# sdat2/mSWE-GNN

Measured on AMD Instinct MI355X. Metric: mesh-nodes x rollout-steps / sec (fine-scale nodes); fp32 max-abs err vs CPU ref, higher is better.
Workload: dtype f32

## Files before the change

### mswe-gnn_amd/build_engine.py

```python
import hashlib
import os
import subprocess
import sys
from concurrent.futures import ThreadPoolExecutor

HERE = os.path.dirname(os.path.abspath(__file__))
ROOT = os.path.dirname(HERE)
SRC = ["csrc/kernels_nt1.hip", "csrc/kernels_nt2.hip", "csrc/kernels_nt4.hip",
       "csrc/kernels_common.hip", "csrc/plan.hip", "csrc/metrics.hip", "csrc/floodmaps.hip", "csrc/series.hip",
       "csrc/train.hip"]
HDR = ["csrc/engine.h", "csrc/kernels_impl.h", "csrc/tiling.h", "csrc/graph_build.h", os.path.join(ROOT, "include", "mswegnn.h")]
HDR += sorted(os.path.join("csrc", "kernels", f) for f in os.listdir(os.path.join(HERE, "csrc", "kernels")) if f.endswith(".h"))
ARCH = os.environ.get("MSW_OFFLOAD_ARCH", "gfx950")
FLAGS = ["-O3", "-std=c++17", "-fPIC", f"--offload-arch={ARCH}", "-Wall", "-Wno-unused-result",
         "-I", os.path.join(ROOT, "include")]


def source_hash(variant=""):
    h = hashlib.sha256()
    for f in SRC + HDR:
        path = f if os.path.isabs(f) else os.path.join(HERE, f)
        h.update(os.path.basename(path).encode())
        with open(path, "rb") as fh:
            h.update(fh.read())
    h.update(" ".join(FLAGS + [variant]).replace(ROOT, "<root>").encode())
    return h.hexdigest()


def lib_path(variant=""):
    return os.path.join(HERE, "lib", f"libmswegnn_{variant}.so" if variant else "libmswegnn.so")


def library_matches_sources(variant=""):
    try:
        with open(lib_path(variant) + ".srchash") as f:
            return f.read().strip() == source_hash(variant)
    except OSError:
        return False


def _newer(a, b):
    return not os.path.exists(b) or os.path.getmtime(a) > os.path.getmtime(b)


def build(force=False, verbose=True, variant=""):
    odir = os.path.join(HERE, "_obj" + (f"_{variant}" if variant else ""))
    extra = {"trace": ["-DMSW_TRACE"],
             "valubase": ["-DMSW_PRELU_MAX=0", "-DMSW_EDGE_FULL=0"],
             "nostream": ["-DMSW_STREAM_ST=0"]}.get(variant, [])
    os.makedirs(odir, exist_ok=True)
    os.makedirs(os.path.join(HERE, "lib"), exist_ok=True)
    out = lib_path(variant)
    if os.path.exists(out) and not library_matches_sources(variant):
        force = True
    objs, cmds = [], []
    hdr_t = max(os.path.getmtime(h if os.path.isabs(h) else os.path.join(HERE, h)) for h in HDR)
    for s in SRC:
        src = os.path.join(HERE, s)
        obj = os.path.join(odir, os.path.basename(s) + ".o")
        objs.append(obj)
        stale = force or _newer(src, obj) or (os.path.exists(obj) and hdr_t > os.path.getmtime(obj))
        if stale:
            cmds.append(["hipcc", *FLAGS, *extra, "-c", src, "-o", obj])
    jobs = max(1, min(len(cmds), int(os.environ.get("MAX_JOBS", os.cpu_count() or 1)), 8))
    with ThreadPoolExecutor(jobs) as ex:
        for cmd in cmds:
            if verbose:
                print(" ".join(cmd), flush=True)
        for r in list(ex.map(lambda c: subprocess.run(c, check=False), cmds)):
            if r.returncode != 0:
                raise subprocess.CalledProcessError(r.returncode, r.args)
    if force or any(_newer(o, out) for o in objs):
        cmd = ["hipcc", f"--offload-arch={ARCH}", "-shared", "-fPIC", "-o", out, *objs]
        if verbose:
            print(" ".join(cmd), flush=True)
        subprocess.run(cmd, check=True)
    with open(out + ".srchash", "w") as f:
        f.write(source_hash(variant) + "\n")
    return out


if __name__ == "__main__":
    var = [a[len("--variant="):] for a in sys.argv if a.startswith("--variant=")]
    build(force="--force" in sys.argv, variant="trace" if "--trace" in sys.argv else (var[0] if var else ""))
```

### mswe-gnn_amd/csrc/kernels/k_base.h

```cpp
#pragma once

__device__ __forceinline__ f32x4 ld4(const float* p) { return *reinterpret_cast<const f32x4*>(p); }
__device__ __forceinline__ void st4(float* p, f32x4 v) { *reinterpret_cast<f32x4*>(p) = v; }
#ifndef MSW_STREAM_ST
#define MSW_STREAM_ST 1
#endif
__device__ __forceinline__ void st4_stream(float* p, f32x4 v) {
  if constexpr (MSW_STREAM_ST)
    __builtin_nontemporal_store(v, reinterpret_cast<f32x4*>(p));
  else
    st4(p, v);
}
__device__ __forceinline__ float hsum(f32x4 v) { return (v.x + v.y) + (v.z + v.w); }
__device__ __forceinline__ f32x4 zero4() { return f32x4{0.f, 0.f, 0.f, 0.f}; }

__device__ __forceinline__ float row_sum(float v) {
  const unsigned u = __float_as_uint(v);
  const auto a = __builtin_amdgcn_permlane16_swap(u, u, false, false);
  const float s = __uint_as_float(a[0]) + __uint_as_float(a[1]);
  const unsigned us = __float_as_uint(s);
  const auto b = __builtin_amdgcn_permlane32_swap(us, us, false, false);
  return __uint_as_float(b[0]) + __uint_as_float(b[1]);
}

template <int NT>
__device__ __forceinline__ void normalize_s(f32x4 (&sv)[NT]) {
#pragma clang fp contract(off)
  float ss = 0.f;
#pragma unroll
  for (int t = 0; t < NT; ++t) ss += hsum(sv[t] * sv[t]);
  const float nrm = sqrtf(row_sum(ss));
#pragma unroll
  for (int t = 0; t < NT; ++t) {
    f32x4 q = sv[t] / nrm;
    q.x = (q.x == q.x) ? q.x : 0.f;
    q.y = (q.y == q.y) ? q.y : 0.f;
    q.z = (q.z == q.z) ? q.z : 0.f;
    q.w = (q.w == q.w) ? q.w : 0.f;
    sv[t] = q;
  }
}

__device__ __forceinline__ int wave_id() { return threadIdx.x >> 6; }
__device__ __forceinline__ int logical_block(const Common& c) {
  const int b = blockIdx.x;
  if (c.xcd <= 0) return b;
  const int x = b % kXcds;
  return x < c.xcd ? (b / kXcds) * c.xcd + x : -1;
}
__device__ __forceinline__ int wave_row0() { return (blockIdx.x * kWaves + wave_id()) * kRowsPerWave; }

#ifndef MSW_PRELU_MAX
#define MSW_PRELU_MAX 1
#endif
template <int ACT>
__device__ __forceinline__ float act_static(float x, float slope) {
  if constexpr (ACT == 1) return MSW_PRELU_MAX ? fmaxf(x, slope * x) : (x > 0.f ? x : slope * x);
  else if constexpr (ACT == 8) return x > 0.f ? x : slope * x;
  else if constexpr (ACT == 2) return x > 0.f ? x : 0.f;
  else if constexpr (ACT == 3) return x > 0.f ? x : 0.1f * x;
  else if constexpr (ACT == 4) return x > 0.f ? x : expm1f(x);
  else if constexpr (ACT == 5) return x / (1.f + expf(-x));
  else if constexpr (ACT == 6) return 1.f / (1.f + expf(-x));
  else if constexpr (ACT == 7) return tanhf(x);
  else return x;
}
template <int ACT, int N>
__device__ __forceinline__ void act_tiles_static(f32x4 (&v)[N], float slope) {
  if constexpr (ACT == 1 && MSW_PRELU_MAX) {
#pragma unroll
    for (int t = 0; t < N; ++t) {
      const f32x4 m = v[t] * slope;
#pragma unroll
      for (int r = 0; r < 4; ++r) v[t][r] = fmaxf(v[t][r], m[r]);
    }
  } else {
#pragma unroll
    for (int t = 0; t < N; ++t)
#pragma unroll
      for (int r = 0; r < 4; ++r) v[t][r] = act_static<ACT>(v[t][r], slope);
  }
}
template <int ACT, int N>
__device__ __forceinline__ void act_tiles(f32x4 (&v)[N], int act, float slope) {
  if constexpr (ACT >= 0) {
    act_tiles_static<ACT, N>(v, slope);
  } else {
    switch (act) {
      case 1: act_tiles_static<8, N>(v, slope); break;
      case 2: act_tiles_static<2, N>(v, slope); break;
      case 3: act_tiles_static<3, N>(v, slope); break;
      case 4: act_tiles_static<4, N>(v, slope); break;
      case 5: act_tiles_static<5, N>(v, slope); break;
      case 6: act_tiles_static<6, N>(v, slope); break;
      case 7: act_tiles_static<7, N>(v, slope); break;
      default: break;
    }
  }
}

template <int ACT, int N>
__device__ __forceinline__ void mask_pad(f32x4 (&v)[N], int fl, int g) {
  if constexpr (ACT < 0) {
#pragma unroll
    for (int t = 0; t < N; ++t)
#pragma unroll
      for (int r = 0; r < 4; ++r) v[t][r] = (16 * t + 4 * g + r < fl) ? v[t][r] : 0.f;
  }
}

template <int TIN, int TOUT>
__device__ __forceinline__ void proj(const f32x4 (&in)[TIN], f32x4 (&acc)[TOUT],
                                     const float* __restrict__ A, int lane) {
#pragma unroll
  for (int to = 0; to < TOUT; ++to) acc[to] = zero4();
#pragma unroll
  for (int ti = 0; ti < TIN; ++ti) {
    f32x4 w[TOUT];
#pragma unroll
    for (int to = 0; to < TOUT; ++to) w[to] = ld4(A + ((size_t)(to * TIN + ti) * 64 + lane) * 4);
#pragma unroll
    for (int r = 0; r < 4; ++r)
#pragma unroll
      for (int to = 0; to < TOUT; ++to) acc[to] = MSW_MFMA(w[to][r], in[ti][r], acc[to]);
  }
}

template <int TIN, int TOUT, int ACT>
__device__ __forceinline__ void mfma_layer(const f32x4 (&in)[TIN], f32x4 (&out)[TOUT],
                                           const LayerDev& L, const float* __restrict__ W,
                                           int lane, int g) {
  f32x4 acc[TOUT];
  proj<TIN, TOUT>(in, acc, W + L.a_off, lane);
#pragma unroll
  for (int to = 0; to < TOUT; ++to) acc[to] = acc[to] + ld4(W + L.b_off + 16 * to + 4 * g);
  act_tiles<ACT, TOUT>(acc, L.act, L.slope);
#pragma unroll
  for (int to = 0; to < TOUT; ++to) out[to] = acc[to];
}

template <int IN0, int T, int TL, int ACT>
__device__ __forceinline__ void run_mlp(const f32x4 (&in)[IN0], f32x4 (&out)[TL], const MlpDev& m,
                                        const float* __restrict__ W, int lane, int g) {
  if (m.n == 1) {
    mfma_layer<IN0, TL, ACT>(in, out, m.l[0], W, lane, g);
    return;
  }
  f32x4 h[T];
  mfma_layer<IN0, T, ACT>(in, h, m.l[0], W, lane, g);
  for (int li = 1; li + 1 < m.n; ++li) {
    f32x4 h2[T];
    mfma_layer<T, T, ACT>(h, h2, m.l[li], W, lane, g);
#pragma unroll
    for (int t = 0; t < T; ++t) h[t] = h2[t];
  }
  mfma_layer<T, TL, ACT>(h, out, m.l[m.n - 1], W, lane, g);
}

template <int N>
__device__ __forceinline__ void load_row(f32x4 (&v)[N], const float* row, int g) {
#pragma unroll
  for (int t = 0; t < N; ++t) v[t] = ld4(row + 16 * t + 4 * g);
}
template <int N, bool STREAM = false>
__device__ __forceinline__ void store_row(float* row, const f32x4 (&v)[N], int ntiles, int g) {
#pragma unroll
  for (int t = 0; t < N; ++t)
    if (t < ntiles) {
      if constexpr (STREAM)
        st4_stream(row + 16 * t + 4 * g, v[t]);
      else
        st4(row + 16 * t + 4 * g, v[t]);
    }
}

template <int NT, int H1T, bool STREAM = false>
__device__ __forceinline__ void np_project_t(const f32x4 (&xs)[NT], const f32x4 (&xin)[NT],
                                             const NpDesc& d, const float* W, size_t n, bool valid,
                                             int lane, int g) {
  constexpr int F = 16 * NT, T2 = 2 * NT;
  f32x4 in[T2];
#pragma unroll
  for (int t = 0; t < NT; ++t) {
    in[t] = xs[t];
    in[NT + t] = xin[t];
  }
  if (d.a_u >= 0) {
    f32x4 acc[H1T];
    proj<T2, H1T>(in, acc, W + d.a_u, lane);
    if (valid) store_row<H1T, STREAM>(d.U + n * (16 * H1T), acc, H1T, g);
  }
  if (d.a_v >= 0) {
    f32x4 acc[H1T];
    proj<T2, H1T>(in, acc, W + d.a_v, lane);
    if (valid) store_row<H1T, STREAM>(d.V + n * (16 * H1T), acc, H1T, g);
  }
  if (d.a_o >= 0) {
    f32x4 acc[NT];
    proj<NT, NT>(xin, acc, W + d.a_o, lane);
    if (valid) store_row<NT, STREAM>(d.O + n * F, acc, NT, g);
  }
}
template <int NT, bool STREAM = false>
__device__ __forceinline__ void np_project(const f32x4 (&xs)[NT], const f32x4 (&xin)[NT],
                                           const NpDesc& d, const float* W, size_t n, bool valid,
                                           int lane, int g) {
  if (d.h1t == 2 * NT)
    np_project_t<NT, 2 * NT, STREAM>(xs, xin, d, W, n, valid, lane, g);
  else
    np_project_t<NT, NT, STREAM>(xs, xin, d, W, n, valid, lane, g);
}

template <int TIN, int H1T, int NT, bool STREAM = false>
__device__ __forceinline__ void side_proj_t(const f32x4 (&in)[TIN], const float* A, float* dst, size_t n,
                                            bool valid, int lane, int g) {
  f32x4 acc[H1T];
  proj<TIN, H1T>(in, acc, A, lane);
  if (valid) store_row<H1T, STREAM>(dst + n * (16 * H1T), acc, H1T, g);
}
template <int TIN, int NT, bool STREAM = false>
__device__ __forceinline__ void side_proj(const f32x4 (&in)[TIN], int h1t, const float* A, float* dst,
                                          size_t n, bool valid, int lane, int g) {
  if (h1t == 2 * NT)
    side_proj_t<TIN, 2 * NT, NT, STREAM>(in, A, dst, n, valid, lane, g);
  else
    side_proj_t<TIN, NT, NT, STREAM>(in, A, dst, n, valid, lane, g);
}

constexpr int kMaxDyn = 16;
template <int NT>
constexpr bool kBcHoist = NT <= 2;
template <int NT>
struct EpiPre {
  f32x4 xs[NT];
  float xd[kMaxDyn];
  int ext, step;
  int bc;
  float bcv[kMaxDyn / 2];
  float bck[kMaxDyn];
};
template <int NT, bool BYCOL = false>
__device__ __forceinline__ void bc_prefetch(EpiPre<NT>& p, const DecDesc& d, const Common& c) {
  const RolloutIO* io = d.io;
  const bool on = p.bc >= 0 && p.step + 1 < io->bc_tstride;
  const float* bp = on ? io->bc + (size_t)p.bc * c.p * io->bc_tstride + p.step + 1 : c.zrow;
  const int ts = on ? io->bc_tstride : 0;
  if constexpr (BYCOL) {
    const int c0 = io->type_bc - 1;
#pragma unroll
    for (int k = 0; k < kMaxDyn; ++k) {
      const int u = (k - c0) >> 1;
      const bool col = k >= c0 && ((k - c0) & 1) == 0 && u < c.p;
      p.bck[k] = bp[col ? u * ts : 0];
    }
  } else {
#pragma unroll
    for (int u = 0; u < kMaxDyn / 2; ++u) p.bcv[u] = u < c.p ? bp[u * ts] : 0.f;
  }
}
template <int NT>
__device__ __forceinline__ void epi_prefetch(EpiPre<NT>& p, const Epilogue& e, const Common& c,
                                             const float* xs_rows, size_t n, int g) {
  constexpr int F = 16 * NT;
  if (e.np.a_u >= 0 || e.np.a_v >= 0 || e.np.a_o >= 0 || e.uu_a >= 0) load_row<NT>(p.xs, xs_rows + n * F, g);
  if (e.dec.on) {
    p.ext = c.perm ? c.perm[n] : (int)n;
    p.step = e.dec.io ? e.dec.io->step : 0;
    p.bc = e.dec.bc_slot ? e.dec.bc_slot[n] : -1;
    const size_t row = e.dec.x_internal ? n : (size_t)(p.ext > 0 ? p.ext : 0);
    const float* xr = e.dec.X + row * c.nnf + (c.nnf - c.dyn);
#pragma unroll
    for (int k = 0; k < kMaxDyn; ++k) p.xd[k] = k < c.dyn ? xr[k] : 0.f;
  }
}
template <int NT>
__device__ __forceinline__ void decode_tail(const f32x4 (&o)[1], const DecDesc& d, const Common& c,
                                            const EpiPre<NT>& pre, int n, bool valid, int g);
template <int NT, int ACT>
__device__ __forceinline__ void decode_rows(const f32x4 (&xup)[NT], const DecDesc& d, const Common& c,
                                            const EpiPre<NT>& pre, int n, bool valid, int lane, int g) {
#pragma clang fp contract(off)
  f32x4 x0[NT], o[1];
#pragma unroll
  for (int t = 0; t < NT; ++t) x0[t] = xup[t];
  act_tiles<-1, NT>(x0, d.pre_act, d.pre_slope);
  run_mlp<NT, NT, 1, ACT>(x0, o, d.dec, c.W, lane, g);
  decode_tail<NT>(o, d, c, pre, n, valid, g);
}
template <int NT>
__device__ __forceinline__ void decode_tail(const f32x4 (&o)[1], const DecDesc& d, const Common& c,
                                            const EpiPre<NT>& pre, int n, bool valid, int g) {
#pragma clang fp contract(off)
  if (!valid || g) return;
  const int ext = pre.ext;
  if (ext < 0) return;
  float* xw = const_cast<float*>(d.X) + (size_t)(d.x_internal ? n : ext) * c.nnf + (c.nnf - c.dyn);
  float h = o[0].x, v = o[0].y;
  if (d.resw_off >= 0) {
    const float* rw = c.W + d.resw_off;
    float rh = pre.xd[0] * rw[0];
    float rv = pre.xd[1] * rw[1];
#pragma unroll
    for (int tau = 1; tau < kMaxDyn / 2; ++tau) {
      if (tau < c.p) {
        rh = rh + pre.xd[2 * tau] * rw[2 * tau];
        rv = rv + pre.xd[2 * tau + 1] * rw[2 * tau + 1];
      }
    }
    h = h + rh;
    v = v + rv;
  }
  h = h > 0.f ? h : 0.f;
  v = v > 0.f ? v : 0.f;
  const float hm = h * (fabsf(h) > 1e-4f ? 1.f : 0.f);
  const float vm = v * (h != 0.f ? 1.f : 0.f);
  if (!d.io) {
    d.y[(size_t)ext * 2 + 0] = hm;
    d.y[(size_t)ext * 2 + 1] = vm;
    return;
  }
  RolloutIO* io = d.io;
  const int t = pre.step;
  io->out[((size_t)ext * 2 + 0) * io->T + t] = hm;
  io->out[((size_t)ext * 2 + 1) * io->T + t] = vm;
#pragma unroll
  for (int k = 0; k + 2 < kMaxDyn; ++k)
    if (k + 2 < c.dyn) xw[k] = pre.xd[k + 2];
  xw[c.dyn - 2] = hm;
  xw[c.dyn - 1] = vm;
  const int b = pre.bc;
  if (b >= 0 && t + 1 < io->bc_tstride) {
    for (int tau = 0; tau < c.p; ++tau)
      xw[(io->type_bc - 1) + 2 * tau] = io->bc[((size_t)b * c.p + tau) * io->bc_tstride + t + 1];
  }
}

template <int NT, bool BYCOL = false>
__device__ __forceinline__ void decode_state_tail(const f32x4 (&o)[1], const DecDesc& d, const Common& c,
                                                  const float* W, const EpiPre<NT>& pre, int n, bool valid,
                                                  int lane, int g, float (&nd)[kMaxDyn]);
template <int NT, int ACT, bool BYCOL = false>
__device__ __forceinline__ void decode_state(const f32x4 (&x)[NT], const DecDesc& d, const Common& c,
                                             const float* W, const EpiPre<NT>& pre, int n, bool valid,
                                             int lane, int g, float (&nd)[kMaxDyn]) {
#pragma clang fp contract(off)
  f32x4 x0[NT], o[1];
#pragma unroll
  for (int t = 0; t < NT; ++t) x0[t] = x[t];
  act_tiles<-1, NT>(x0, d.pre_act, d.pre_slope);
  run_mlp<NT, NT, 1, ACT>(x0, o, d.dec, W, lane, g);
  decode_state_tail<NT, BYCOL>(o, d, c, W, pre, n, valid, lane, g, nd);
}
template <int NT, bool BYCOL>
__device__ __forceinline__ void decode_state_tail(const f32x4 (&o)[1], const DecDesc& d, const Common& c,
                                                  const float* W, const EpiPre<NT>& pre, int n, bool valid,
                                                  int lane, int g, float (&nd)[kMaxDyn]) {
#pragma clang fp contract(off)
  float h = __shfl(o[0].x, lane & 15), v = __shfl(o[0].y, lane & 15);
  if (d.resw_off >= 0) {
    const float* rw = W + d.resw_off;
    float rh = pre.xd[0] * rw[0];
    float rv = pre.xd[1] * rw[1];
#pragma unroll
    for (int tau = 1; tau < kMaxDyn / 2; ++tau) {
      if (tau < c.p) {
        rh = rh + pre.xd[2 * tau] * rw[2 * tau];
        rv = rv + pre.xd[2 * tau + 1] * rw[2 * tau + 1];
      }
    }
    h = h + rh;
    v = v + rv;
  }
  h = h > 0.f ? h : 0.f;
  v = v > 0.f ? v : 0.f;
  const float hm = h * (fabsf(h) > 1e-4f ? 1.f : 0.f);
  const float vm = v * (h != 0.f ? 1.f : 0.f);
  const RolloutIO* io = d.io;
  const int t = pre.step, b = pre.bc;
  const bool bc_on = b >= 0 && t + 1 < io->bc_tstride;
  const int c0 = io->type_bc - 1;
#pragma unroll
  for (int k = 0; k < kMaxDyn; ++k) {
    float val = k + 2 < c.dyn ? pre.xd[k + 2] : (k == c.dyn - 2 ? hm : (k == c.dyn - 1 ? vm : 0.f));
    const int tau = (k - c0) >> 1;
    float bv;
    if constexpr (BYCOL) {
      bv = pre.bck[k];
    } else {
      bv = 0.f;
#pragma unroll
      for (int u = 0; u < kMaxDyn / 2; ++u) bv = u == tau ? pre.bcv[u] : bv;
    }
    if (bc_on && k >= c0 && ((k - c0) & 1) == 0 && tau < c.p) val = bv;
    nd[k] = val;
  }
  if (!valid || g || pre.ext < 0) return;
  const int ext = pre.ext;
  io->out[((size_t)ext * 2 + 0) * io->T + t] = hm;
  io->out[((size_t)ext * 2 + 1) * io->T + t] = vm;
  float* xw = const_cast<float*>(d.X) + (size_t)n * c.nnf + (c.nnf - c.dyn);
#pragma unroll
  for (int k = 0; k < kMaxDyn; ++k)
    if (k < c.dyn) xw[k] = nd[k];
}

__device__ __forceinline__ float nd_column(const float (&nd)[kMaxDyn], int g, int q, int dyn) {
  static_assert(kMaxDyn == 16, "four lane groups x four columns");
  const float v = g == 0 ? nd[q] : g == 1 ? nd[4 + q] : g == 2 ? nd[8 + q] : nd[12 + q];
  return 4 * g + q < dyn ? v : 0.f;
}

template <int NT, int ACT>
__device__ __forceinline__ void node_epilogue(f32x4 (&res)[NT], const Epilogue& e, const Common& c,
                                              const EpiPre<NT>& pre, float* out, int n,
                                              bool valid, int lane, int g) {
  constexpr int F = 16 * NT, T2 = 2 * NT;
  if (e.post_act) {
    act_tiles<-1, NT>(res, e.post_act, e.post_slope);
    mask_pad<ACT, NT>(res, c.fl, g);
  }
  if (out && valid) store_row<NT>(out + (size_t)n * F, res, NT, g);
  const bool np = e.np.a_u >= 0 || e.np.a_v >= 0 || e.np.a_o >= 0;
  if (np || e.uu_a >= 0) {
    const f32x4(&xs)[NT] = pre.xs;
    if (np) np_project<NT>(xs, res, e.np, c.W, n, valid, lane, g);
    if (e.uu_a >= 0) {
      f32x4 in[T2];
#pragma unroll
      for (int t = 0; t < NT; ++t) {
        in[t] = xs[t];
        in[NT + t] = res[t];
      }
      side_proj<T2, NT>(in, e.uu_h1t, c.W + e.uu_a, e.Uu, n, valid, lane, g);
    }
  }
  if (e.dec.on) decode_rows<NT, ACT>(res, e.dec, c, pre, n, valid, lane, g);
}

#ifdef MSW_TRACE
constexpr int kTraceWG = 8192;
#define MSW_MARK(c, k)                                                          \
  do {                                                                          \
    if ((c).trace && blockIdx.x == 0 && threadIdx.x < 64) {                     \
      __builtin_amdgcn_s_waitcnt(0);                                            \
      const unsigned long long t0 = __builtin_amdgcn_s_memtime();               \
      const unsigned long long t1 = __builtin_amdgcn_s_memrealtime();           \
      if (threadIdx.x == 0) { (c).trace[2 * (k)] = t0; (c).trace[2 * (k) + 1] = t1; } \
    }                                                                           \
    if ((c).trace && (k) == 0 && threadIdx.x == 0 && blockIdx.x < kTraceWG)     \
      (c).trace[32 + 2 * blockIdx.x] = __builtin_amdgcn_s_memrealtime();       \
    if ((c).trace && (k) == 9 && blockIdx.x < kTraceWG) {                       \
      __builtin_amdgcn_s_waitcnt(0);                                            \
      const unsigned long long te = __builtin_amdgcn_s_memrealtime();           \
      if ((threadIdx.x & 63) == 0) atomicMax(&(c).trace[33 + 2 * blockIdx.x], te); \
    }                                                                           \
  } while (0)
#else
#define MSW_MARK(c, k) \
  do {                 \
  } while (0)
#endif

template <int WV = kWaves>
__device__ __forceinline__ void stage_glds(float* smem, const float* __restrict__ W, WReg r, int first, int last) {
  const int lane = threadIdx.x & 63;
  for (int ch = first / kChunk + wave_id(); ch * kChunk < last; ch += WV)
    __builtin_amdgcn_global_load_lds(
        (const __attribute__((address_space(1))) void*)(W + r.off + ch * kChunk + lane * 4),
        (__attribute__((address_space(3))) void*)(smem + ch * kChunk), 16, 0, 0);
}
__device__ __forceinline__ int chunk_ceil(int n) { return (n + kChunk - 1) / kChunk * kChunk; }
```

### mswe-gnn_amd/csrc/kernels/k_coop_edge.h

```cpp
#pragma once

template <int N, int TS>
__device__ __forceinline__ f32x4 pick(const f32x4 (&a)[N], int r, int t) {
  f32x4 v = a[t];
#pragma unroll
  for (int k = 1; k < N / TS; ++k) v = (r == k) ? a[k * TS + t] : v;
  return v;
}
template <int T, int P>
__device__ __forceinline__ void coop_exchange(const f32x4* sub, f32x4 (&full)[T], float* buf, int xw, int r,
                                              int j, int g) {
  constexpr int TS = T / P;
#pragma unroll
  for (int t = 0; t < TS; ++t) st4(buf + j * xw + 16 * (r * TS + t) + 4 * g, sub[t]);
  __syncthreads();
#pragma unroll
  for (int t = 0; t < T; ++t) full[t] = ld4(buf + j * xw + 16 * t + 4 * g);
}
template <int TIN, int TS, int ACT>
__device__ __forceinline__ void mfma_layer_sub(const f32x4 (&in)[TIN], f32x4 (&out)[TS], const LayerDev& L,
                                               const float* __restrict__ W, int to0, int lane, int g) {
  f32x4 acc[TS];
  proj<TIN, TS>(in, acc, W + L.a_off + (size_t)to0 * TIN * 256, lane);
#pragma unroll
  for (int to = 0; to < TS; ++to) acc[to] = acc[to] + ld4(W + L.b_off + 16 * (to0 + to) + 4 * g);
  act_tiles<ACT, TS>(acc, L.act, L.slope);
#pragma unroll
  for (int to = 0; to < TS; ++to) out[to] = acc[to];
}
template <int TIN, int TS>
struct LayerOps {
  f32x4 w[TIN][TS];
  f32x4 b[TS];
};
template <int TIN, int TS>
__device__ __forceinline__ void ops_load(LayerOps<TIN, TS>& o, const LayerDev& L, const float* __restrict__ W,
                                         int to0, int lane, int g) {
  const float* A = W + L.a_off + (size_t)to0 * TIN * 256;
#pragma unroll
  for (int ti = 0; ti < TIN; ++ti)
#pragma unroll
    for (int to = 0; to < TS; ++to) o.w[ti][to] = ld4(A + ((size_t)(to * TIN + ti) * 64 + lane) * 4);
#pragma unroll
  for (int to = 0; to < TS; ++to) o.b[to] = ld4(W + L.b_off + 16 * (to0 + to) + 4 * g);
}
template <int TIN, int TS, int ACT>
__device__ __forceinline__ void ops_layer(const f32x4 (&in)[TIN], f32x4 (&out)[TS], const LayerOps<TIN, TS>& o,
                                          const LayerDev& L) {
  f32x4 acc[TS];
#pragma unroll
  for (int to = 0; to < TS; ++to) acc[to] = zero4();
#pragma unroll
  for (int ti = 0; ti < TIN; ++ti)
#pragma unroll
    for (int r = 0; r < 4; ++r)
#pragma unroll
      for (int to = 0; to < TS; ++to) acc[to] = MSW_MFMA(o.w[ti][to][r], in[ti][r], acc[to]);
#pragma unroll
  for (int to = 0; to < TS; ++to) acc[to] = acc[to] + o.b[to];
  act_tiles<ACT, TS>(acc, L.act, L.slope);
#pragma unroll
  for (int to = 0; to < TS; ++to) out[to] = acc[to];
}
template <int TIN, int TOUT, int D>
__device__ __forceinline__ void proj_ahead(const f32x4 (&in)[TIN], f32x4 (&acc)[TOUT], const float* __restrict__ A,
                                           int lane) {
  static_assert(D >= 1 && D <= TIN, "prefetch depth");
  f32x4 w[D][TOUT];
#pragma unroll
  for (int d = 0; d < D; ++d)
#pragma unroll
    for (int to = 0; to < TOUT; ++to) w[d][to] = ld4(A + ((size_t)(to * TIN + d) * 64 + lane) * 4);
#pragma unroll
  for (int to = 0; to < TOUT; ++to) acc[to] = zero4();
#pragma unroll
  for (int ti = 0; ti < TIN; ++ti) {
    f32x4 cur[TOUT];
#pragma unroll
    for (int to = 0; to < TOUT; ++to) cur[to] = w[ti % D][to];
    if (ti + D < TIN) {
#pragma unroll
      for (int to = 0; to < TOUT; ++to) w[ti % D][to] = ld4(A + ((size_t)(to * TIN + ti + D) * 64 + lane) * 4);
    }
#pragma unroll
    for (int r = 0; r < 4; ++r)
#pragma unroll
      for (int to = 0; to < TOUT; ++to) acc[to] = MSW_MFMA(cur[to][r], in[ti][r], acc[to]);
  }
}
template <int IN0, int T, int TL, int ACT, int P>
__device__ __forceinline__ void coop_run_mlp(const f32x4 (&in)[IN0], f32x4 (&out)[TL], const MlpDev& m,
                                             const float* __restrict__ W, int lane, int g, int j, int r,
                                             float* buf0, float* buf1, int xw) {
  if (m.n == 1) {
    f32x4 o[TL / P];
    mfma_layer_sub<IN0, TL / P, ACT>(in, o, m.l[0], W, r * (TL / P), lane, g);
    coop_exchange<TL, P>(o, out, buf0, xw, r, j, g);
    return;
  }
  f32x4 h[T];
  {
    f32x4 o[T / P];
    mfma_layer_sub<IN0, T / P, ACT>(in, o, m.l[0], W, r * (T / P), lane, g);
    coop_exchange<T, P>(o, h, buf0, xw, r, j, g);
  }
  for (int li = 1; li + 1 < m.n; ++li) {
    f32x4 o[T / P];
    mfma_layer_sub<T, T / P, ACT>(h, o, m.l[li], W, r * (T / P), lane, g);
    coop_exchange<T, P>(o, h, (li & 1) ? buf1 : buf0, xw, r, j, g);
  }
  f32x4 o[TL / P];
  mfma_layer_sub<T, TL / P, ACT>(h, o, m.l[m.n - 1], W, r * (TL / P), lane, g);
  coop_exchange<TL, P>(o, out, ((m.n - 1) & 1) ? buf1 : buf0, xw, r, j, g);
}
template <int TIN, int TS, int D = 0>
__device__ __forceinline__ void proj_store_part(const f32x4 (&in)[TIN], const float* A, int r, float* dst, size_t n,
                                                int ntl, bool valid, int lane, int g) {
  f32x4 acc[TS];
  if constexpr (D > 0)
    proj_ahead<TIN, TS, (D < TIN ? D : TIN)>(in, acc, A + (size_t)r * TS * TIN * 256, lane);
  else
    proj<TIN, TS>(in, acc, A + (size_t)r * TS * TIN * 256, lane);
  if (valid) {
#pragma unroll
    for (int t = 0; t < TS; ++t) st4(dst + n * (16 * ntl) + 16 * (r * TS + t) + 4 * g, acc[t]);
  }
}
template <int NT, int H1T, int P, int D = 0>
__device__ __forceinline__ void np_project_coop(const f32x4 (&xs)[NT], const f32x4 (&xin)[NT], const NpDesc& d,
                                                const float* W, size_t n, bool valid, int r, int lane, int g) {
  constexpr int T2 = 2 * NT;
  f32x4 in[T2];
#pragma unroll
  for (int t = 0; t < NT; ++t) {
    in[t] = xs[t];
    in[NT + t] = xin[t];
  }
  if (d.a_u >= 0) proj_store_part<T2, H1T / P, D>(in, W + d.a_u, r, d.U, n, H1T, valid, lane, g);
  if (d.a_v >= 0) proj_store_part<T2, H1T / P, D>(in, W + d.a_v, r, d.V, n, H1T, valid, lane, g);
  if constexpr (P <= NT) {
    if (d.a_o >= 0) proj_store_part<NT, NT / P, D>(xin, W + d.a_o, r, d.O, n, NT, valid, lane, g);
  } else {
    if (d.a_o >= 0 && r < NT) proj_store_part<NT, 1, D>(xin, W + d.a_o, r, d.O, n, NT, valid, lane, g);
  }
}

template <int NT>
struct PoolIn {
  f32x4 c[kPoolInline][NT];
  f32x4 xs[NT];
  int cnt, off;
};
template <int NT, int LST>
__device__ __forceinline__ void edge_pool_load(EdgeHopRows<NT>& r, PoolIn<NT>& pi, const EdgeHopArgs& a, int tile,
                                               int j, int g, int rank) {
  constexpr int F = 16 * NT, T2 = 2 * NT;
  const LaneRec rec = load_rec(a.recs, tile, j);
  const int4* sp = reinterpret_cast<const int4*>(a.pool.slots + (size_t)tile * kRowsPerWave + j) + (rank ? 2 : 0);
  const int4 r0 = sp[0], r1 = sp[1];
  r.L = lanes_of(rec, tile, j, a.n0);
  const Lanes& L = r.L;
  const int hs = 16 * a.h1t;
  const float* z = a.c.zrow;
  const float* Pb = a.Pe ? a.Pe + L.p * hs : z;
#pragma unroll
  for (int t = 0; t < T2; ++t) r.Ps[t] = ld4((t < a.h1t ? Pb : z) + 16 * t + 4 * g);
  const int ci[kPoolInline] = {r0.x, r0.y, r0.z, r0.w};
#pragma unroll
  for (int k = 0; k < kPoolInline; ++k) load_row<NT>(pi.c[k], a.pool.in + (size_t)ci[k] * F, g);
  pi.cnt = r1.x; pi.off = r1.y;
  load_row<NT>(pi.xs, a.xs + (rank ? L.n : L.sr) * F, g);
  load_row<NT>(r.sk, a.skip ? a.skip + L.n * F : z, g);
  if (LST && a.last) epi_prefetch<NT>(r.pre, a.epi, a.c, a.xs, L.n, g);
}
template <int NT>
__device__ __forceinline__ void pool_mean(f32x4 (&m)[NT], const PoolIn<NT>& pi, const EdgeHopArgs& a, int g) {
#pragma clang fp contract(off)
  constexpr int F = 16 * NT;
#pragma unroll
  for (int t = 0; t < NT; ++t) m[t] = zero4();
#pragma unroll
  for (int k = 0; k < kPoolInline; ++k)
#pragma unroll
    for (int t = 0; t < NT; ++t) {
      const f32x4 s2 = m[t] + pi.c[k][t];
      m[t] = k < pi.cnt ? s2 : m[t];
    }
  for (int k = kPoolInline; k < pi.cnt; ++k) {
    f32x4 y[NT];
    load_row<NT>(y, a.pool.in + (size_t)a.pool.child[pi.off + k] * F, g);
#pragma unroll
    for (int t = 0; t < NT; ++t) m[t] = m[t] + y[t];
  }
  const float fc = (float)(pi.cnt > 0 ? pi.cnt : 1);
#pragma unroll
  for (int t = 0; t < NT; ++t) m[t] = m[t] / fc;
}
template <int NT, int H1T>
__device__ __forceinline__ void pool_project_t(f32x4 (&h)[2 * NT], f32x4 (&o)[NT], const f32x4 (&xp)[NT],
                                               const f32x4 (&xs)[NT], const NpDesc& d, const float* W, int lane,
                                               int rank) {
  constexpr int T2 = 2 * NT;
  f32x4 in[T2], acc[H1T];
#pragma unroll
  for (int t = 0; t < NT; ++t) {
    in[t] = xs[t];
    in[NT + t] = xp[t];
  }
  proj<T2, H1T>(in, acc, W + (rank ? d.a_v : d.a_u), lane);
#pragma unroll
  for (int t = 0; t < T2; ++t) h[t] = t < H1T ? acc[t < H1T ? t : 0] : zero4();
  if (d.a_o >= 0) {
    proj<NT, NT>(xp, o, W + d.a_o, lane);
  } else {
#pragma unroll
    for (int t = 0; t < NT; ++t) o[t] = xp[t];
  }
}
template <int NT, int XS>
__device__ __forceinline__ void side_project_exchange(EdgeHopRows<NT>& q, const f32x4 (&xp)[NT], const f32x4 (&xs)[NT],
                                                      const NpDesc& np, const float* W, int lane, int g, int j,
                                                      int rank, float* pb, float* slab0, float* slab1) {
  constexpr int T2 = 2 * NT;
  f32x4 h[T2], o[NT];
  if (np.h1t == T2)
    pool_project_t<NT, T2>(h, o, xp, xs, np, W, lane, rank);
  else
    pool_project_t<NT, NT>(h, o, xp, xs, np, W, lane, rank);
  if (rank == 0) {
    store_row<T2>(pb + j * XS, h, T2, g);
    store_row<NT>(pb + j * XS + 16 * T2, o, NT, g);
  } else {
    store_row<T2>(slab0 + j * XS, h, T2, g);
    store_row<NT>(slab0 + j * XS + 16 * T2, o, NT, g);
    store_row<T2>(slab1 + j * XS, h, T2, g);
    store_row<NT>(slab1 + j * XS + 16 * T2, o, NT, g);
  }
  __syncthreads();
  if (rank == 0) {
#pragma unroll
    for (int t = 0; t < T2; ++t) q.Us[t] = h[t];
#pragma unroll
    for (int t = 0; t < NT; ++t) q.os[t] = o[t];
    load_row<NT>(q.inn, slab0 + j * XS + 16 * T2, g);
  } else {
    load_row<T2>(q.Us, pb + j * XS, g);
    load_row<NT>(q.os, pb + j * XS + 16 * T2, g);
#pragma unroll
    for (int t = 0; t < NT; ++t) q.inn[t] = o[t];
  }
}

template <int NT>
struct UnpoolIn {
  f32x4 uc[2 * NT], vv[2 * NT];
  f32x4 xc[NT], sk[NT], xs[NT];
  bool ev;
};
template <int NT, int LST>
__device__ __forceinline__ void edge_unpool_load(EdgeHopRows<NT>& r, UnpoolIn<NT>& u, const EdgeHopArgs& a, int tile,
                                                 int j, int g, int rank) {
  constexpr int F = 16 * NT, T2 = 2 * NT;
  const PoolFuse& d = a.pool;
  const LaneRec rec = load_rec(a.recs, tile, j);
  const int2 pp = d.parent[(size_t)tile * kRowsPerWave + j];
  r.L = lanes_of(rec, tile, j, a.n0);
  const Lanes& L = r.L;
  const float* z = a.c.zrow;
  {
    const int hs = 16 * a.h1t;
    const float* Pb = a.Pe ? a.Pe + L.p * hs : z;
#pragma unroll
    for (int t = 0; t < T2; ++t) r.Ps[t] = ld4((t < a.h1t ? Pb : z) + 16 * t + 4 * g);
  }
  const size_t v = rank ? L.n : L.sr;
  const int pc = rank ? pp.y : pp.x;
  u.ev = pc >= 0;
  const size_t c = (size_t)(pc >= 0 ? pc : d.cpad);
  const int hs = 16 * d.h1t;
#pragma unroll
  for (int t = 0; t < T2; ++t) {
    const bool on = t < d.h1t;
    u.uc[t] = ld4((on ? d.Uu + c * hs : z) + 16 * t + 4 * g);
    u.vv[t] = ld4((on ? d.Vu + v * hs : z) + 16 * t + 4 * g);
  }
  load_row<NT>(u.xc, d.xc + c * F, g);
  load_row<NT>(u.sk, d.skip ? d.skip + v * F : z, g);
  load_row<NT>(u.xs, a.xs + v * F, g);
  load_row<NT>(r.sk, a.skip ? a.skip + L.n * F : z, g);
  if (LST && a.last) epi_prefetch<NT>(r.pre, a.epi, a.c, a.xs, L.n, g);
}
template <int NT>
__device__ __forceinline__ void unpool_row(f32x4 (&res)[NT], const UnpoolIn<NT>& u, const EdgeHopArgs& a,
                                           const float* W, int lane, int g) {
#pragma clang fp contract(off)
  constexpr int T2 = 2 * NT;
  const PoolFuse& d = a.pool;
  f32x4 H[T2];
  const int b1 = d.b1_off >= 0 ? d.b1_off : 0;
#pragma unroll
  for (int t = 0; t < T2; ++t) {
    const f32x4 br = ld4(W + b1 + 16 * t + 4 * g);
    H[t] = (t < d.h1t) ? (u.uc[t] + u.vv[t]) + br : zero4();
  }
  act_tiles<-1, T2>(H, d.act1, d.slope1);
  f32x4 sv[NT];
  if (d.rest.n > 0) {
    run_mlp<T2, T2, NT, -1>(H, sv, d.rest, W, lane, g);
  } else {
#pragma unroll
    for (int t = 0; t < NT; ++t) sv[t] = H[t];
  }
  if (d.normalize) normalize_s<NT>(sv);
  float rs = 0.f, rd = 0.f;
#pragma unroll
  for (int t = 0; t < NT; ++t) {
    rs += hsum(u.xc[t]);
    rd += hsum(zero4());
  }
  const bool act = (row_sum(rs) != 0.f) || (row_sum(rd) != 0.f);
#pragma unroll
  for (int t = 0; t < NT; ++t) {
    f32x4 gv;
    if (d.grad) {
      gv = zero4() - u.xc[t];
      if (d.upwind) {
        gv.x = gv.x < 0.f ? 0.f : gv.x; gv.y = gv.y < 0.f ? 0.f : gv.y;
        gv.z = gv.z < 0.f ? 0.f : gv.z; gv.w = gv.w < 0.f ? 0.f : gv.w;
      }
    } else {
      gv = u.xc[t];
    }
    const f32x4 m = gv * sv[t];
    const f32x4 agg = zero4() + ((u.ev && act) ? m : zero4());
    res[t] = (zero4() + agg) + u.sk[t];
  }
  if (d.post_act) act_tiles<-1, NT>(res, d.post_act, d.post_slope);
}

template <int NT, int ACT, int LST, int P, int FUSE = 0>
__global__ __launch_bounds__(64 * kWaves) void k_edge_coop(EdgeHopArgs a) {
#pragma clang fp contract(off)
  constexpr int F = 16 * NT, T2 = 2 * NT;
  constexpr int XS = 16 * 2 * NT + 16 * NT + 4;
  constexpr int XW = 16 * T2 + 4;
  constexpr int G = kWaves / P;
  __shared__ __attribute__((aligned(16))) float slab_all[kWaves][kRowsPerWave][XS];
  __shared__ __attribute__((aligned(16))) float xbuf[G][2][kRowsPerWave][XW];
  __shared__ __attribute__((aligned(16))) float pbuf[FUSE ? G : 1][kRowsPerWave][XS];
  extern __shared__ __attribute__((aligned(16))) float smem[];
  const int lane = threadIdx.x & 63, g = lane >> 4, j = lane & 15, w = wave_id();
  const int grp = w / P, r = w % P;
  const int xb = logical_block(a.c);
  if (xb < 0) return;
  const int tile = xb * G + grp;
  const bool live = tile < a.ntiles;
  Common c = a.c;
  if (a.step_inc && blockIdx.x == 0 && threadIdx.x == 0) *a.step_inc += 1;
  f32x4 wf[NT][NT];
  load_filter<NT>(wf, a.c.W, a.filt_a, lane);
  auto body = [&](auto full) __attribute__((always_inline)) {
    constexpr bool FULL = decltype(full)::value;
    EdgeHopRows<NT> q;
    [[maybe_unused]] PoolIn<NT> pin;
    [[maybe_unused]] UnpoolIn<NT> uin;
    if constexpr (FUSE == 1)
      edge_pool_load<NT, LST>(q, pin, a, live ? tile : 0, j, g, r);
    else if constexpr (FUSE == 2)
      edge_unpool_load<NT, LST>(q, uin, a, live ? tile : 0, j, g, r);
    else
      edge_hop_load<NT, LST, FULL>(q, a, live ? tile : 0, j, g);
    const bool split = a.reg.split < a.reg_nf;
    stage_glds<kWaves>(smem, a.c.W, a.reg, 0, a.reg.split);
    __syncthreads();
    c.W = smem;
    if (split) stage_glds<kWaves>(smem, a.c.W, a.reg, chunk_ceil(a.reg.split), a.reg_nf);
    if constexpr (FUSE != 0) {
      static_assert(P == 2, "fused pooling / unpooling: a source rank and a destination rank");
      f32x4 xp[NT];
      if constexpr (FUSE == 1)
        pool_mean<NT>(xp, pin, a, g);
      else
        unpool_row<NT>(xp, uin, a, c.W, lane, g);
      side_project_exchange<NT, XS>(q, xp, FUSE == 1 ? pin.xs : uin.xs, a.pool.np, c.W, lane, g, j, r,
                                    &pbuf[grp][0][0], &slab_all[grp * P][0][0], &slab_all[grp * P + 1][0][0]);
    }
    float* slab = &slab_all[w][0][0];
    float* b0 = &xbuf[grp][0][0][0];
    float* b1p = &xbuf[grp][1][0][0];
    const Lanes& L = q.L;
    float* my = slab + j * XS;
    if constexpr (FUSE == 0) {
      store_row<T2>(my, q.Vn, T2, g);
      store_row<NT>(my + 16 * T2, q.inn, NT, g);
      wave_lds_sync();
    }
    const float* dr = slab + L.dl * XS;
    f32x4 H[T2], od[NT];
    const int b1 = a.b1_off >= 0 ? a.b1_off : 0;
    f32x4 vr[T2], br[T2];
#pragma unroll
    for (int t = 0; t < T2; ++t) {
      const int off = 16 * t + 4 * g;
      vr[t] = ld4(dr + off);
      if constexpr (!FULL) br[t] = ld4(c.W + b1 + off);
    }
#pragma unroll
    for (int t = 0; t < T2; ++t) {
      if constexpr (FULL) {
        H[t] = (q.Us[t] + vr[t]) + q.Ps[t];
      } else {
        const f32x4 p = a.Pe ? q.Ps[t] : br[t];
        H[t] = (t < a.h1t) ? (q.Us[t] + vr[t]) + p : zero4();
      }
    }
    load_row<NT>(od, dr + 16 * T2, g);
    act_tiles<ACT, T2>(H, a.act1, a.slope1);
    f32x4 sv[NT];
    if (a.rest.n > 0) {
      coop_run_mlp<T2, T2, NT, ACT, P>(H, sv, a.rest, c.W, lane, g, j, r, b0, b1p, XW);
    } else {
#pragma unroll
      for (int t = 0; t < NT; ++t) sv[t] = H[t];
    }
    mask_pad<ACT, NT>(sv, a.c.fl, g);
    if (a.normalize) normalize_s<NT>(sv);
    if (live && r == 0 && a.s) store_row<NT>(a.s + L.p * F, sv, NT, g);
    put_message<NT, FULL ? 1 : -1>(my, q.os, od, sv, L.ev, a.grad, a.upwind, g);
    f32x4 agg[NT];
    gather_messages<NT, XS>(agg, slab, L.q0, L.q1, g);
    constexpr int TS = NT / P;
    f32x4 rs[TS];
#pragma unroll
    for (int t = 0; t < TS; ++t) rs[t] = pick<NT, TS>(q.inn, r, t);
    if (a.filt_a >= 0) {
      f32x4 wr[TS][NT];
#pragma unroll
      for (int to = 0; to < TS; ++to)
#pragma unroll
        for (int ti = 0; ti < NT; ++ti) {
          f32x4 v = wf[to][ti];
#pragma unroll
          for (int k = 1; k < P; ++k) v = (r == k) ? wf[k * TS + to][ti] : v;
          wr[to][ti] = v;
        }
      f32x4 acc[TS];
#pragma unroll
      for (int to = 0; to < TS; ++to) acc[to] = zero4();
#pragma unroll
      for (int ti = 0; ti < NT; ++ti)
#pragma unroll
        for (int rr = 0; rr < 4; ++rr)
#pragma unroll
          for (int to = 0; to < TS; ++to) acc[to] = MSW_MFMA(wr[to][ti][rr], agg[ti][rr], acc[to]);
#pragma unroll
      for (int t = 0; t < TS; ++t) rs[t] = rs[t] + acc[t];
    } else {
#pragma unroll
      for (int t = 0; t < TS; ++t) rs[t] = rs[t] + pick<NT, TS>(agg, r, t);
    }
    if constexpr (!FULL) {
      if (a.skip) {
#pragma unroll
        for (int t = 0; t < TS; ++t) rs[t] = rs[t] + pick<NT, TS>(q.sk, r, t);
      }
    }
    f32x4 res[NT];
    coop_exchange<NT, P>(rs, res, (a.rest.n & 1) ? b1p : b0, XW, r, j, g);
    if (split) __syncthreads();
    if (LST && a.last) {
      const Epilogue& e = a.epi;
      if (e.post_act) {
        act_tiles<-1, NT>(res, e.post_act, e.post_slope);
        mask_pad<ACT, NT>(res, a.c.fl, g);
      }
      if (live && r == 0 && a.out && L.nv) store_row<NT>(a.out + L.n * F, res, NT, g);
      if (e.np.h1t == T2)
        np_project_coop<NT, T2, P>(q.pre.xs, res, e.np, c.W, L.n, live && L.nv, r, lane, g);
      else
        np_project_coop<NT, NT, P>(q.pre.xs, res, e.np, c.W, L.n, live && L.nv, r, lane, g);
    } else if (live && r == 0 && L.nv && a.out) {
      store_row<NT>(a.out + L.n * F, res, NT, g);
    }
  };
  if (edge_full(a, NT))
    body(std::true_type{});
  else
    body(std::false_type{});
}

template <int NT, int P, int H1T>
__device__ __forceinline__ void pool_project_part(float* dst_row, const f32x4 (&xp)[NT], const f32x4 (&xs)[NT],
                                                  const NpDesc& d, const float* W, int lane, int g, int side,
                                                  int part) {
  constexpr int NPART = P / 2, T2 = 2 * NT, TU = H1T / NPART, TO = NT / NPART;
  static_assert(H1T % NPART == 0 && NT % NPART == 0, "whole output tiles per rank");
  f32x4 in[T2], acc[TU];
#pragma unroll
  for (int t = 0; t < NT; ++t) {
    in[t] = xs[t];
    in[NT + t] = xp[t];
  }
  proj<T2, TU>(in, acc, W + (side ? d.a_v : d.a_u) + (size_t)part * TU * T2 * 256, lane);
#pragma unroll
  for (int t = 0; t < TU; ++t) st4(dst_row + 16 * (part * TU + t) + 4 * g, acc[t]);
  if (part == 0)
#pragma unroll
    for (int t = H1T; t < T2; ++t) st4(dst_row + 16 * t + 4 * g, zero4());
  f32x4 o[TO];
  if (d.a_o >= 0) {
    proj<NT, TO>(xp, o, W + d.a_o + (size_t)part * TO * NT * 256, lane);
  } else {
#pragma unroll
    for (int t = 0; t < TO; ++t) o[t] = pick<NT, TO>(xp, part, t);
  }
#pragma unroll
  for (int t = 0; t < TO; ++t) st4(dst_row + 16 * T2 + 16 * (part * TO + t) + 4 * g, o[t]);
}

template <int ACT, int LST, int P = 4, int FUSE = 0>
__global__ __launch_bounds__(64 * kWaves) void k_edge_coop4(EdgeHopArgs a) {
#pragma clang fp contract(off)
  static_assert(FUSE == 0 || FUSE == 1, "k_edge_coop4: plain or fused pooling");
  constexpr int NT = 4, F = 16 * NT, T2 = 2 * NT, G = kWaves / P, TS = NT / P;
  constexpr int XS = 16 * 2 * NT + 16 * NT + 4;
  constexpr int XW = 16 * T2 + 4;
  __shared__ __attribute__((aligned(16))) float slab_g[G][kRowsPerWave][XS];
  __shared__ __attribute__((aligned(16))) float xbuf_g[G][2][kRowsPerWave][XW];
  extern __shared__ __attribute__((aligned(16))) float smem[];
  const int lane = threadIdx.x & 63, g = lane >> 4, j = lane & 15, w = wave_id();
  const int grp = w / P, r = w % P;
  const int xb = logical_block(a.c);
  if (xb < 0) return;
  const int tile0 = xb * G + grp;
  const bool live = tile0 < a.ntiles;
  const int tile = live ? tile0 : 0;
  float (&slab)[kRowsPerWave][XS] = slab_g[grp];
  float (&xbuf)[2][kRowsPerWave][XW] = xbuf_g[grp];
  Common c = a.c;
  if (a.step_inc && blockIdx.x == 0 && threadIdx.x == 0) *a.step_inc += 1;
  f32x4 wr[TS][NT];
  {
    const int fa = a.filt_a >= 0 ? a.filt_a : 0;
#pragma unroll
    for (int t = 0; t < TS; ++t)
#pragma unroll
      for (int ti = 0; ti < NT; ++ti) wr[t][ti] = ld4(c.W + fa + ((size_t)((r * TS + t) * NT + ti) * 64 + lane) * 4);
  }
  const bool full = edge_full(a, NT);
  EdgeHopRows<NT> q;
  [[maybe_unused]] PoolIn<NT> pin;
  [[maybe_unused]] const int side = r >= P / 2;
  if constexpr (FUSE == 1)
    edge_pool_load<NT, LST>(q, pin, a, tile, j, g, side);
  else if (full)
    edge_hop_load<NT, LST, true>(q, a, tile, j, g);
  else
    edge_hop_load<NT, LST>(q, a, tile, j, g);
  const Lanes& L = q.L;
  if (a.reg.len > 0 && !a.wdirect) stage_glds<kWaves>(smem, c.W, a.reg, 0, a.reg.len);
  auto rest = [&](const float* Wm, auto fullc) __attribute__((always_inline)) {
    constexpr bool FULL = decltype(fullc)::value;
    float* my = &slab[j][0];
    if constexpr (FUSE != 0) {
      constexpr int XPB = 16 * T2 + 16 * NT + 4;
      static_assert(kRowsPerWave * XPB <= 2 * kRowsPerWave * XW, "exchange rows fit the xbuf pair");
      float* pb = &xbuf[0][0][0] + j * XPB;
      f32x4 xp[NT];
      pool_mean<NT>(xp, pin, a, g);
      const f32x4(&xsr)[NT] = pin.xs;
      if (a.pool.np.h1t == T2)
        pool_project_part<NT, P, T2>(side ? my : pb, xp, xsr, a.pool.np, c.W, lane, g, side, r % (P / 2));
      else
        pool_project_part<NT, P, NT>(side ? my : pb, xp, xsr, a.pool.np, c.W, lane, g, side, r % (P / 2));
      __syncthreads();
      load_row<T2>(q.Us, pb, g);
      load_row<NT>(q.os, pb + 16 * T2, g);
    } else if (r == 0) {
      store_row<T2>(my, q.Vn, T2, g);
      store_row<NT>(my + 16 * T2, q.inn, NT, g);
    }
    __syncthreads();
    const float* dr = &slab[L.dl][0];
    f32x4 H[T2], od[NT];
    const int b1 = a.b1_off >= 0 ? a.b1_off : 0;
    f32x4 vr[T2], br[T2];
#pragma unroll
    for (int t = 0; t < T2; ++t) {
      const int off = 16 * t + 4 * g;
      vr[t] = ld4(dr + off);
      if constexpr (!FULL) br[t] = ld4(Wm + b1 + off);
    }
#pragma unroll
    for (int t = 0; t < T2; ++t) {
      if constexpr (FULL) {
        H[t] = (q.Us[t] + vr[t]) + q.Ps[t];
      } else {
        const f32x4 p = a.Pe ? q.Ps[t] : br[t];
        H[t] = (t < a.h1t) ? (q.Us[t] + vr[t]) + p : zero4();
      }
    }
    load_row<NT>(od, dr + 16 * T2, g);
    act_tiles<ACT, T2>(H, a.act1, a.slope1);
    f32x4 sv[NT];
    if (a.rest.n > 0) {
      coop_run_mlp<T2, T2, NT, ACT, P>(H, sv, a.rest, Wm, lane, g, j, r, &xbuf[0][0][0], &xbuf[1][0][0], XW);
    } else {
#pragma unroll
      for (int t = 0; t < NT; ++t) sv[t] = H[t];
    }
    mask_pad<ACT, NT>(sv, a.c.fl, g);
    if (a.normalize) normalize_s<NT>(sv);
    if (live && r == 0 && a.s) store_row<NT>(a.s + L.p * F, sv, NT, g);
    if (a.rest.n == 0) __syncthreads();
    if (r == 0) put_message<NT, FULL ? 1 : -1>(my, q.os, od, sv, L.ev, a.grad, a.upwind, g);
    __syncthreads();
    f32x4 agg[NT];
    gather_messages<NT, XS>(agg, &slab[0][0], L.q0, L.q1, g);
    f32x4 rs[TS];
#pragma unroll
    for (int t = 0; t < TS; ++t) rs[t] = ld4(&slab[j][16 * T2 + 16 * (r * TS + t) + 4 * g]);
    if (a.filt_a >= 0) {
      f32x4 acc[TS];
#pragma unroll
      for (int t = 0; t < TS; ++t) acc[t] = zero4();
#pragma unroll
      for (int ti = 0; ti < NT; ++ti)
#pragma unroll
        for (int rr = 0; rr < 4; ++rr)
#pragma unroll
          for (int t = 0; t < TS; ++t) acc[t] = MSW_MFMA(wr[t][ti][rr], agg[ti][rr], acc[t]);
#pragma unroll
      for (int t = 0; t < TS; ++t) rs[t] = rs[t] + acc[t];
    } else {
#pragma unroll
      for (int t = 0; t < TS; ++t) {
        f32x4 ag = zero4();
        for (int qq = L.q0; qq < L.q1; ++qq) ag = ag + ld4(&slab[qq][16 * (r * TS + t) + 4 * g]);
        rs[t] = rs[t] + ag;
      }
    }
    if (!FULL && a.skip) {
#pragma unroll
      for (int t = 0; t < TS; ++t) rs[t] = rs[t] + ld4(a.skip + L.n * F + 16 * (r * TS + t) + 4 * g);
    }
    f32x4 res[NT];
    coop_exchange<NT, P>(rs, res, (a.rest.n & 1) ? &xbuf[1][0][0] : &xbuf[0][0][0], XW, r, j, g);
    if (LST && a.last) {
      const Epilogue& e = a.epi;
      if (e.post_act) {
        act_tiles<-1, NT>(res, e.post_act, e.post_slope);
        mask_pad<ACT, NT>(res, a.c.fl, g);
      }
      if (live && r == 0 && a.out && L.nv) store_row<NT>(a.out + L.n * F, res, NT, g);
      if (e.np.h1t == T2)
        np_project_coop<NT, T2, P>(q.pre.xs, res, e.np, c.W, L.n, L.nv && live, r, lane, g);
      else
        np_project_coop<NT, NT, P>(q.pre.xs, res, e.np, c.W, L.n, L.nv && live, r, lane, g);
    } else if (live && r == 0 && L.nv && a.out) {
      store_row<NT>(a.out + L.n * F, res, NT, g);
    }
  };
  auto run = [&](auto fullc) __attribute__((always_inline)) {
    if constexpr (P == 4) {
      if (a.reg.len > 0 && !a.wdirect)
        rest((const float*)smem, fullc);
      else
        rest(a.reg.len > 0 ? c.W + a.reg.off : c.W, fullc);
    } else {
      rest(a.reg.len > 0 ? (a.wdirect ? c.W + a.reg.off : (const float*)smem) : c.W, fullc);
    }
  };
  if (full)
    run(std::true_type{});
  else
    run(std::false_type{});
}

template <int NT>
static const void* edge_coop_kernel(int prelu, int last, int pw = 0, int pool = 0) {
  if constexpr (NT == 2) {
    if (pool == 1) {
      if (last) return prelu ? (const void*)k_edge_coop<NT, 1, 1, 2, 1> : (const void*)k_edge_coop<NT, -1, 1, 2, 1>;
      return prelu ? (const void*)k_edge_coop<NT, 1, 0, 2, 1> : (const void*)k_edge_coop<NT, -1, 0, 2, 1>;
    }
    if (pool == 2) {
      if (last) return prelu ? (const void*)k_edge_coop<NT, 1, 1, 2, 2> : (const void*)k_edge_coop<NT, -1, 1, 2, 2>;
      return prelu ? (const void*)k_edge_coop<NT, 1, 0, 2, 2> : (const void*)k_edge_coop<NT, -1, 0, 2, 2>;
    }
    if (last) return prelu ? (const void*)k_edge_coop<NT, 1, 1, 2> : (const void*)k_edge_coop<NT, -1, 1, 2>;
    return prelu ? (const void*)k_edge_coop<NT, 1, 0, 2> : (const void*)k_edge_coop<NT, -1, 0, 2>;
  } else if constexpr (NT == 4) {
    if (pool == 1) {
      if (pw == 2) {
        if (last) return prelu ? (const void*)k_edge_coop4<1, 1, 2, 1> : (const void*)k_edge_coop4<-1, 1, 2, 1>;
        return prelu ? (const void*)k_edge_coop4<1, 0, 2, 1> : (const void*)k_edge_coop4<-1, 0, 2, 1>;
      }
      if (last) return prelu ? (const void*)k_edge_coop4<1, 1, 4, 1> : (const void*)k_edge_coop4<-1, 1, 4, 1>;
      return prelu ? (const void*)k_edge_coop4<1, 0, 4, 1> : (const void*)k_edge_coop4<-1, 0, 4, 1>;
    }
    if (pool == 2) return nullptr;
    if (pw == 2) {
      if (last) return prelu ? (const void*)k_edge_coop4<1, 1, 2> : (const void*)k_edge_coop4<-1, 1, 2>;
      return prelu ? (const void*)k_edge_coop4<1, 0, 2> : (const void*)k_edge_coop4<-1, 0, 2>;
    }
    if (last) return prelu ? (const void*)k_edge_coop4<1, 1> : (const void*)k_edge_coop4<-1, 1>;
    return prelu ? (const void*)k_edge_coop4<1, 0> : (const void*)k_edge_coop4<-1, 0>;
  }
  return nullptr;
}
```

### mswe-gnn_amd/csrc/kernels/k_coop_encode.h

```cpp
#pragma once

template <int IN0, int T, int TL, int ACT, int P, int XW>
__device__ __forceinline__ void enc_coop_mlp(const f32x4 (&in)[IN0], f32x4 (&out)[TL], const MlpDev& m,
                                             const float* __restrict__ W, int lane, int g, int j, int r,
                                             float* buf, int& xc) {
  static_assert(T % P == 0, "hidden tiles split evenly over the ranks");
  auto last = [&](const auto& h) {
    constexpr int TI = sizeof(h) / sizeof(f32x4);
    if constexpr (TL % P == 0) {
      f32x4 o[TL / P];
      mfma_layer_sub<TI, TL / P, ACT>(h, o, m.l[m.n - 1], W, r * (TL / P), lane, g);
      coop_exchange<TL, P>(o, out, buf + (xc++ & 1) * kRowsPerWave * XW, XW, r, j, g);
    } else {
      mfma_layer<TI, TL, ACT>(h, out, m.l[m.n - 1], W, lane, g);
    }
  };
  if (m.n == 1) {
    last(in);
    return;
  }
  f32x4 h[T];
  {
    f32x4 o[T / P];
    mfma_layer_sub<IN0, T / P, ACT>(in, o, m.l[0], W, r * (T / P), lane, g);
    coop_exchange<T, P>(o, h, buf + (xc++ & 1) * kRowsPerWave * XW, XW, r, j, g);
  }
  for (int li = 1; li + 1 < m.n; ++li) {
    f32x4 o[T / P];
    mfma_layer_sub<T, T / P, ACT>(h, o, m.l[li], W, r * (T / P), lane, g);
    coop_exchange<T, P>(o, h, buf + (xc++ & 1) * kRowsPerWave * XW, XW, r, j, g);
  }
  last(h);
}
template <int IN0, int T, int TL, int ACT, int P, int XW>
struct CoopMlp {
  static constexpr int TS = T / P;
  static constexpr bool XL = TL % P == 0;
  static constexpr bool PF = (XL ? TL / P : TL) == TS;
  LayerOps<IN0, TS> first;
  __device__ __forceinline__ void load(const MlpDev& m, const float* __restrict__ W, int r, int lane, int g) {
    if constexpr (PF) ops_load<IN0, TS>(first, m.l[0], W, (m.n == 1 && !XL) ? 0 : r * TS, lane, g);
  }
  template <class Hook>
  __device__ __forceinline__ void run(const f32x4 (&in)[IN0], f32x4 (&out)[TL], const MlpDev& m,
                                      const float* __restrict__ W, int lane, int g, int j, int r, float* buf,
                                      int& xc, Hook&& hook) const {
    if constexpr (!PF) {
      hook();
      enc_coop_mlp<IN0, T, TL, ACT, P, XW>(in, out, m, W, lane, g, j, r, buf, xc);
    } else {
      const int tl0 = XL ? r * TS : 0;
      auto finish = [&](const f32x4 (&o)[TS]) {
        if constexpr (XL) {
          coop_exchange<TL, P>(o, out, buf + (xc++ & 1) * kRowsPerWave * XW, XW, r, j, g);
        } else {
#pragma unroll
          for (int t = 0; t < TL; ++t) out[t] = o[t];
        }
      };
      f32x4 o[TS];
      if (m.n == 1) {
        ops_layer<IN0, TS, ACT>(in, o, first, m.l[0]);
        hook();
        finish(o);
        return;
      }
      LayerOps<T, TS> nx;
      ops_load<T, TS>(nx, m.l[1], W, m.n == 2 ? tl0 : r * TS, lane, g);
      ops_layer<IN0, TS, ACT>(in, o, first, m.l[0]);
      hook();
      f32x4 h[T];
      coop_exchange<T, P>(o, h, buf + (xc++ & 1) * kRowsPerWave * XW, XW, r, j, g);
      ops_layer<T, TS, ACT>(h, o, nx, m.l[1]);
      for (int li = 2; li < m.n; ++li) {
        coop_exchange<T, P>(o, h, buf + (xc++ & 1) * kRowsPerWave * XW, XW, r, j, g);
        LayerOps<T, TS> cur;
        ops_load<T, TS>(cur, m.l[li], W, li + 1 == m.n ? tl0 : r * TS, lane, g);
        ops_layer<T, TS, ACT>(h, o, cur, m.l[li]);
      }
      finish(o);
    }
  }
};
constexpr int kEncProjAhead = 4;
template <int NT> constexpr int enc_coop_waves() { return NT == 2 ? 8 : kWaves; }
template <int NT, int ACT, bool DEC, int P, int WV = enc_coop_waves<NT>()>
__global__ __launch_bounds__(64 * WV) __attribute__((amdgpu_waves_per_eu(4))) void k_encode_coop(EncodeArgs a) {
  constexpr int F = 16 * NT, T2 = 2 * NT, G = WV / P;
  constexpr int XW = 16 * T2 + 4;
  __shared__ __attribute__((aligned(16))) float xbuf[G][2][kRowsPerWave][XW];
  extern __shared__ __attribute__((aligned(16))) float smem[];
  const int lane = threadIdx.x & 63, g = lane >> 4, j = lane & 15, w = wave_id();
  const int grp = w / P, r = w % P;
  MSW_MARK(a.c, 0);
  Common c = a.c;
  const int dstep = DEC ? a.dec.io->step : -1;
  if (!a.dec.on && a.io && blockIdx.x == 0 && threadIdx.x == 0) a.io->step += 1;
  const int rb = blockIdx.x * (G * kRowsPerWave);
  int s = 0;
  while (s + 1 < a.S && rb >= a.n0[s + 1]) ++s;
  const int n = rb + grp * kRowsPerWave + j;
  const bool valid = (n - a.n0[s]) < a.ns[s];
  const int ext = a.c.perm ? a.c.perm[n] : n;
  const int xrow = a.x_internal ? (valid ? n : a.n0[s]) : (valid ? ext : 0);
  const float* xr = a.x + (size_t)xrow * a.c.nnf;
  const int nstat = a.c.nstat_raw;
  float raw[4], dyn[4];
  float wlv;
  EpiPre<NT> pre;
  constexpr int DS = NT / P;
  f32x4 xu[DS];
  if (DEC) {
#pragma unroll
    for (int t = 0; t < DS; ++t) xu[t] = ld4(a.dec_in + (size_t)n * F + 16 * (r * DS + t) + 4 * g);
    pre.ext = ext;
    pre.bc = a.dec.bc_slot[n];
#pragma unroll
    for (int k = 0; k < kMaxDyn; ++k) pre.xd[k] = k < c.dyn ? xr[nstat + k] : 0.f;
  }
#pragma unroll
  for (int q = 0; q < 4; ++q) {
    const int f = 4 * g + q;
    raw[q] = f < nstat ? xr[f] : 0.f;
    dyn[q] = f < a.c.dyn ? xr[nstat + f] : 0.f;
  }
  wlv = xr[nstat - 1] + xr[a.c.nnf - 2];
  if constexpr (kBcHoist<NT>) {
    if (DEC && dstep >= 0) {
      pre.step = dstep;
      bc_prefetch<NT>(pre, a.dec, c);
    }
  }
  MSW_MARK(c, 1);
  if constexpr (kStaged<NT>) {
    stage_glds<WV>(smem, a.c.W, a.sreg[s], 0, a.sreg[s].len);
    __syncthreads();
  }
  const float* Wl = kStaged<NT> ? (const float*)smem : c.W;
  float* buf = &xbuf[grp][0][0][0];
  int xc = 0;
  CoopMlp<1, NT, NT, ACT, P, XW> stat_mlp, dyn_mlp;
  auto enc_loads = [&]() {
    stat_mlp.load(a.stat, Wl, r, lane, g);
    dyn_mlp.load(a.dynm, Wl, r, lane, g);
  };
  auto none = [&]() {};
  const bool decode = DEC && dstep >= 0;
  if (!decode) enc_loads();
  if (decode) {
#pragma clang fp contract(off)
    CoopMlp<NT, NT, 1, ACT, P, XW> dec_mlp;
    dec_mlp.load(a.dec.dec, Wl, r, lane, g);
    if constexpr (!kBcHoist<NT>) {
      pre.step = dstep;
      bc_prefetch<NT>(pre, a.dec, c);
    }
    float nd[kMaxDyn];
    {
      f32x4 x0[NT], o[1];
      act_tiles<-1, DS>(xu, a.dec.pre_act, a.dec.pre_slope);
      coop_exchange<NT, P>(xu, x0, buf + (xc++ & 1) * kRowsPerWave * XW, XW, r, j, g);
      dec_mlp.run(x0, o, a.dec.dec, Wl, lane, g, j, r, buf, xc, enc_loads);
      decode_state_tail<NT>(o, a.dec, c, Wl, pre, n, valid && r == 0, lane, g, nd);
    }
#pragma unroll
    for (int q = 0; q < 4; ++q) dyn[q] = nd_column(nd, g, q, c.dyn);
    float hn = 0.f;
#pragma unroll
    for (int k = 0; k < kMaxDyn; ++k) hn = (k == c.dyn - 2) ? nd[k] : hn;
    wlv = xr[nstat - 1] + hn;
  }
  if (DEC && a.decode_only) return;
  MSW_MARK(c, 2);
  f32x4 xs[NT];
  {
    f32x4 v;
#pragma unroll
    for (int q = 0; q < 4; ++q) v[q] = (c.with_wl && 4 * g + q == nstat) ? wlv : raw[q];
    const f32x4 in[1] = {v};
    stat_mlp.run(in, xs, a.stat, Wl, lane, g, j, r, buf, xc, none);
    mask_pad<ACT, NT>(xs, c.fl, g);
    if (valid && r == 0) store_row<NT>(a.xs + (size_t)n * F, xs, NT, g);
  }
  MSW_MARK(c, 5);
  if (s == 0) {
    f32x4 xd[NT];
    const f32x4 in[1] = {f32x4{dyn[0], dyn[1], dyn[2], dyn[3]}};
    dyn_mlp.run(in, xd, a.dynm, Wl, lane, g, j, r, buf, xc, none);
    mask_pad<ACT, NT>(xd, c.fl, g);
    if (valid && r == P - 1 && a.xd) store_row<NT>(a.xd + (size_t)n * F, xd, NT, g);
    MSW_MARK(c, 6);
    if (a.np0.h1t == T2)
      np_project_coop<NT, T2, P, kEncProjAhead>(xs, xd, a.np0, Wl, n, valid, r, lane, g);
    else
      np_project_coop<NT, NT, P, kEncProjAhead>(xs, xd, a.np0, Wl, n, valid, r, lane, g);
  }
  MSW_MARK(c, 8);
  if (a.vu_a[s] >= 0) {
    if (a.vu_h1t == T2)
      proj_store_part<NT, T2 / P, kEncProjAhead>(xs, Wl + a.vu_a[s], r, a.Vu, n, T2, valid, lane, g);
    else
      proj_store_part<NT, NT / P, kEncProjAhead>(xs, Wl + a.vu_a[s], r, a.Vu, n, NT, valid, lane, g);
  }
  MSW_MARK(c, 9);
}
```

### mswe-gnn_amd/csrc/kernels/k_edge.h

```cpp
#pragma once

struct Lanes {
  bool ev, nv;
  int dl, q0, q1;
  size_t sr, n;
  size_t p;
};
__device__ __forceinline__ Lanes lanes_of(const LaneRec& r, int tile, int j, int n0) {
  Lanes L;
  L.ev = r.src >= 0;
  L.nv = r.n >= 0;
  L.dl = L.ev ? r.dl : 0;
  L.sr = (size_t)(L.ev ? r.src : n0);
  L.n = (size_t)(L.nv ? r.n : n0);
  L.q0 = r.q & 255;
  L.q1 = L.nv ? (r.q >> 8) : L.q0;
  L.p = (size_t)tile * kRowsPerWave + j;
  return L;
}
__device__ __forceinline__ LaneRec load_rec(const LaneRec* recs, int tile, int j) {
  const int4 v = reinterpret_cast<const int4*>(recs)[(size_t)tile * kRowsPerWave + j];
  return LaneRec{v.x, v.y, v.z, v.w};
}

template <int NT, int GM = -1>
__device__ __forceinline__ void put_message(float* slab_row, const f32x4 (&os)[NT], const f32x4 (&od)[NT],
                                            const f32x4 (&sv)[NT], bool ev, int grad_rt, int upwind_rt, int g) {
#pragma clang fp contract(off)
  const int grad = GM == 1 ? 1 : grad_rt, upwind = GM == 1 ? 0 : upwind_rt;
  float rs = 0.f, rd = 0.f;
#pragma unroll
  for (int t = 0; t < NT; ++t) {
    rs += hsum(os[t]);
    rd += hsum(od[t]);
  }
  const bool act = (row_sum(rs) != 0.f) || (row_sum(rd) != 0.f);
#pragma unroll
  for (int t = 0; t < NT; ++t) {
    f32x4 gv;
    if (grad) {
      gv = od[t] - os[t];
      if (upwind) {
        gv.x = gv.x < 0.f ? 0.f : gv.x; gv.y = gv.y < 0.f ? 0.f : gv.y;
        gv.z = gv.z < 0.f ? 0.f : gv.z; gv.w = gv.w < 0.f ? 0.f : gv.w;
      }
    } else {
      gv = os[t];
    }
    const f32x4 m = gv * sv[t];
    st4(slab_row + 16 * t + 4 * g, (ev && act) ? m : zero4());
  }
}

__device__ __forceinline__ void wave_lds_sync() {
  __builtin_amdgcn_s_waitcnt(0xc07f);
  __builtin_amdgcn_wave_barrier();
}

template <int NT, int STRIDE>
__device__ __forceinline__ void gather_messages(f32x4 (&agg)[NT], const float* slab, int q0, int q1, int g) {
#pragma clang fp contract(off)
  wave_lds_sync();
#pragma unroll
  for (int t = 0; t < NT; ++t) agg[t] = zero4();
  for (int q = q0; q < q1; ++q) {
#pragma unroll
    for (int t = 0; t < NT; ++t) agg[t] = agg[t] + ld4(slab + q * STRIDE + 16 * t + 4 * g);
  }
}

template <int NT>
__device__ __forceinline__ void apply_filter(f32x4 (&res)[NT], const f32x4 (&agg)[NT], int filt_a,
                                             const float* W, int lane) {
#pragma clang fp contract(off)
  if (filt_a >= 0) {
    f32x4 acc[NT];
    proj<NT, NT>(agg, acc, W + filt_a, lane);
#pragma unroll
    for (int t = 0; t < NT; ++t) res[t] = res[t] + acc[t];
  } else {
#pragma unroll
    for (int t = 0; t < NT; ++t) res[t] = res[t] + agg[t];
  }
}

__device__ __forceinline__ int opaque_lane() {
  int ln = (int)(threadIdx.x & 63);
  asm volatile("" : "+v"(ln));
  return ln;
}

template <int NT>
__device__ __forceinline__ void load_filter(f32x4 (&wf)[NT][NT], const float* W, int filt_a, int lane) {
  const int fa = filt_a >= 0 ? filt_a : 0;
#pragma unroll
  for (int to = 0; to < NT; ++to)
#pragma unroll
    for (int ti = 0; ti < NT; ++ti) wf[to][ti] = ld4(W + fa + ((size_t)(to * NT + ti) * 64 + lane) * 4);
}
template <int NT>
__device__ __forceinline__ void apply_filter_regs(f32x4 (&res)[NT], const f32x4 (&agg)[NT], int filt_a,
                                                  const f32x4 (&wf)[NT][NT]) {
#pragma clang fp contract(off)
  if (filt_a >= 0) {
    f32x4 acc[NT];
#pragma unroll
    for (int to = 0; to < NT; ++to) acc[to] = zero4();
#pragma unroll
    for (int ti = 0; ti < NT; ++ti)
#pragma unroll
      for (int r = 0; r < 4; ++r)
#pragma unroll
        for (int to = 0; to < NT; ++to) acc[to] = MSW_MFMA(wf[to][ti][r], agg[ti][r], acc[to]);
#pragma unroll
    for (int t = 0; t < NT; ++t) res[t] = res[t] + acc[t];
  } else {
#pragma unroll
    for (int t = 0; t < NT; ++t) res[t] = res[t] + agg[t];
  }
}

template <int NT>
struct EdgeHopRows {
  Lanes L;
  f32x4 Us[2 * NT], Ps[2 * NT], Vn[2 * NT], os[NT], inn[NT], sk[NT];
  EpiPre<NT> pre;
};
#ifndef MSW_EDGE_FULL
#define MSW_EDGE_FULL 1
#endif
__device__ __forceinline__ bool edge_full(const EdgeHopArgs& a, int nt) {
  return MSW_EDGE_FULL && a.h1t == 2 * nt && a.Pe && !a.own_zero && !a.skip && a.grad && !a.upwind;
}
template <int NT, int LST, bool FULL = false>
__device__ __forceinline__ void edge_hop_gather(EdgeHopRows<NT>& r, const EdgeHopArgs& a, const LaneRec& rec,
                                                int tile, int j, int g) {
  constexpr int F = 16 * NT, T2 = 2 * NT;
  r.L = lanes_of(rec, tile, j, a.n0);
  const Lanes& L = r.L;
  const int hs = FULL ? 16 * T2 : 16 * a.h1t;
  const float* z = a.c.zrow;
  const float* Ub = a.U + L.sr * hs;
  const float* Vb = a.V + L.n * hs;
  const float* Pb = FULL ? a.Pe + L.p * hs : a.Pe ? a.Pe + L.p * hs : z;
#pragma unroll
  for (int t = 0; t < T2; ++t) {
    const int off = 16 * t + 4 * g;
    const bool on = FULL || t < a.h1t;
    r.Us[t] = ld4((on ? Ub : z) + off);
    r.Vn[t] = ld4((on ? Vb : z) + off);
    r.Ps[t] = ld4((on ? Pb : z) + off);
  }
  load_row<NT>(r.os, a.in + L.sr * F, g);
  load_row<NT>(r.inn, !FULL && a.own_zero ? z : a.in + L.n * F, g);
  if constexpr (!FULL) load_row<NT>(r.sk, a.skip ? a.skip + L.n * F : z, g);
  if (LST && a.last) epi_prefetch<NT>(r.pre, a.epi, a.c, a.xs, L.n, g);
}
template <int NT, int LST, bool FULL = false>
__device__ __forceinline__ void edge_hop_load(EdgeHopRows<NT>& r, const EdgeHopArgs& a, int tile, int j, int g) {
  edge_hop_gather<NT, LST, FULL>(r, a, load_rec(a.recs, tile, j), tile, j, g);
}
template <int NT, int ACT, int XS, bool FREG = true, bool FULL = false>
__device__ __forceinline__ void edge_hop_core(const EdgeHopRows<NT>& r, const EdgeHopArgs& a, const Common& c,
                                              const float* Wm, const f32x4 (&wf)[NT][NT], float* slab, int j,
                                              int lane, int g, f32x4 (&res_out)[NT]) {
#pragma clang fp contract(off)
  constexpr int F = 16 * NT, T2 = 2 * NT;
  const Lanes& L = r.L;
  float* my = slab + j * XS;
  store_row<T2>(my, r.Vn, T2, g);
  store_row<NT>(my + 16 * T2, r.inn, NT, g);
  wave_lds_sync();
  const float* dr = slab + L.dl * XS;
  f32x4 H[T2], od[NT];
  const int b1 = a.b1_off >= 0 ? a.b1_off : 0;
  f32x4 vr[T2], br[T2];
#pragma unroll
  for (int t = 0; t < T2; ++t) {
    const int off = 16 * t + 4 * g;
    vr[t] = ld4(dr + off);
    if constexpr (!FULL) br[t] = ld4(Wm + b1 + off);
  }
#pragma unroll
  for (int t = 0; t < T2; ++t) {
    if constexpr (FULL) {
      H[t] = (r.Us[t] + vr[t]) + r.Ps[t];
    } else {
      const f32x4 p = a.Pe ? r.Ps[t] : br[t];
      H[t] = (t < a.h1t) ? (r.Us[t] + vr[t]) + p : zero4();
    }
  }
  load_row<NT>(od, dr + 16 * T2, g);
  MSW_MARK(c, 4);
  act_tiles<ACT, T2>(H, a.act1, a.slope1);
  f32x4 sv[NT];
  if (a.rest.n > 0) {
    run_mlp<T2, T2, NT, ACT>(H, sv, a.rest, Wm, lane, g);
  } else {
#pragma unroll
    for (int t = 0; t < NT; ++t) sv[t] = H[t];
  }
  MSW_MARK(c, 5);
  mask_pad<ACT, NT>(sv, c.fl, g);
  if (a.normalize) normalize_s<NT>(sv);
  if (a.s) store_row<NT>(a.s + L.p * F, sv, NT, g);
  put_message<NT, FULL ? 1 : -1>(my, r.os, od, sv, L.ev, a.grad, a.upwind, g);
  MSW_MARK(c, 6);
  f32x4 agg[NT], res[NT];
  gather_messages<NT, XS>(agg, slab, L.q0, L.q1, g);
  MSW_MARK(c, 7);
#pragma unroll
  for (int t = 0; t < NT; ++t) res[t] = r.inn[t];
  if constexpr (FREG)
    apply_filter_regs<NT>(res, agg, a.filt_a, wf);
  else
    apply_filter<NT>(res, agg, a.filt_l, c.W, lane);
  MSW_MARK(c, 8);
  if constexpr (!FULL) {
    if (a.skip) {
#pragma unroll
      for (int t = 0; t < NT; ++t) res[t] = res[t] + r.sk[t];
    }
  }
#pragma unroll
  for (int t = 0; t < NT; ++t) res_out[t] = res[t];
}
template <int NT, int ACT, int LST>
__device__ __forceinline__ void edge_hop_finish(f32x4 (&res)[NT], const EdgeHopRows<NT>& r, const EdgeHopArgs& a,
                                                const Common& c, int lane, int g) {
  constexpr int F = 16 * NT;
  const Lanes& L = r.L;
  if (LST && a.last) {
    node_epilogue<NT, ACT>(res, a.epi, c, r.pre, a.out, L.n, L.nv, lane, g);
  } else if (L.nv && a.out) {
    store_row<NT>(a.out + L.n * F, res, NT, g);
  }
}
template <int NT, int ACT, bool LOOP, int LST>
__global__ __launch_bounds__((64 * edge_waves<NT, LOOP, LST>())) __attribute__((amdgpu_waves_per_eu(edge_eu<NT, LOOP, LST>())))
void k_edge_hop(EdgeHopArgs a) {
  constexpr int WV = edge_waves<NT, LOOP, LST>();
  constexpr int XS = 16 * 2 * NT + 16 * NT + 4;
  __shared__ __attribute__((aligned(16))) float slab[WV][kRowsPerWave][XS];
  extern __shared__ __attribute__((aligned(16))) float smem[];
  const int lane = threadIdx.x & 63, g = lane >> 4, j = lane & 15, w = wave_id();
  const int stride = gridDim.x * WV;
  const int xb = logical_block(a.c);
  if (xb < 0) return;
  int tile = xb * WV + w;
  Common c = a.c;
  MSW_MARK(c, 0);
  if (a.step_inc && blockIdx.x == 0 && threadIdx.x == 0) *a.step_inc += 1;
  f32x4 wf[NT][NT];
  if constexpr (!LOOP || !kStaged<NT>)
    load_filter<NT>(wf, a.c.W, a.filt_a, lane);
  if constexpr (!LOOP) {
    auto body = [&](auto full) __attribute__((always_inline)) {
      constexpr bool FULL = decltype(full)::value;
      const bool live = tile < a.ntiles;
      EdgeHopRows<NT> r;
      edge_hop_load<NT, LST, FULL>(r, a, live ? tile : 0, j, g);
      MSW_MARK(c, 1);
      const bool split = kStaged<NT> && a.reg.split < a.reg_nf;
      const float* Wm = c.W;
      if constexpr (kStaged<NT>) {
        stage_glds<WV>(smem, a.c.W, a.reg, 0, a.reg.split);
        __syncthreads();
        c.W = smem;
        Wm = smem;
        if (split) stage_glds<WV>(smem, a.c.W, a.reg, chunk_ceil(a.reg.split), a.reg_nf);
      } else if (a.reg.len > 0) {
        stage_glds<WV>(smem, a.c.W, a.reg, 0, a.reg.len);
        __syncthreads();
        Wm = smem;
      }
      MSW_MARK(c, 2);
      f32x4 res[NT];
      if (!kStaged<NT> && a.reg.len > 0) {
        if (live) edge_hop_core<NT, ACT, XS, true, FULL>(r, a, c, (const float*)smem, wf, &slab[w][0][0], j, lane, g, res);
      } else if (live) {
        edge_hop_core<NT, ACT, XS, true, FULL>(r, a, c, Wm, wf, &slab[w][0][0], j, lane, g, res);
      }
      if (split) __syncthreads();
      if (live) edge_hop_finish<NT, ACT, LST>(res, r, a, c, lane, g);
    };
    if (edge_full(a, NT))
      body(std::true_type{});
    else
      body(std::false_type{});
  } else {
    const float* Wm = c.W;
    if constexpr (kStaged<NT>) {
      stage_glds<WV>(smem, a.c.W, a.reg, 0, a.reg.len);
      __syncthreads();
      c.W = smem;
      Wm = smem;
    } else if (a.reg.len > 0) {
      stage_glds<WV>(smem, a.c.W, a.reg, 0, a.reg.len);
      __syncthreads();
      Wm = smem;
    }
    auto walk = [&](const float* Wl, auto full) __attribute__((always_inline)) {
      constexpr bool FULL = decltype(full)::value;
      for (; tile < a.ntiles; tile += stride) {
        const int ln = opaque_lane(), gg = ln >> 4, jj = ln & 15;
        EdgeHopRows<NT> q;
        edge_hop_load<NT, LST, FULL>(q, a, tile, jj, gg);
        f32x4 res[NT];
        edge_hop_core<NT, ACT, XS, !kStaged<NT>, FULL>(q, a, c, Wl, wf, &slab[w][0][0], jj, ln, gg, res);
        edge_hop_finish<NT, ACT, LST>(res, q, a, c, ln, gg);
      }
    };
    const bool full = edge_full(a, NT);
    if (!kStaged<NT> && a.reg.len > 0) {
      if (full)
        walk((const float*)smem, std::true_type{});
      else
        walk((const float*)smem, std::false_type{});
    } else if (full) {
      walk(Wm, std::true_type{});
    } else {
      walk(Wm, std::false_type{});
    }
  }
  MSW_MARK(c, 9);
}

constexpr int kMlpWaves = 8;
template <int NT>
struct MlpFetch {
  f32x4 u[2 * NT], v[2 * NT], p[2 * NT];
  int4 e;
};
template <int NT>
__device__ __forceinline__ void mlp_fetch_full(MlpFetch<NT>& f, const EdgeHopArgs& a, int ch, bool ok, int j, int g) {
  constexpr int T2 = 2 * NT, hs = 16 * T2;
  f.e = reinterpret_cast<const int4*>(a.chunks)[(size_t)ch * kRowsPerWave + j];
  const bool ev = ok && f.e.z >= 0;
  const float* z = a.c.zrow;
  const float* Ub = ok ? a.U + (size_t)(ev ? f.e.x : a.n0) * hs : z;
  const float* Vb = ok ? a.V + (size_t)(ev ? f.e.y : a.n0) * hs : z;
  const float* Pb = ev ? a.Pe + (size_t)f.e.z * hs : z;
#pragma unroll
  for (int t = 0; t < T2; ++t) {
    const int off = 16 * t + 4 * g;
    f.u[t] = ld4(Ub + off);
    f.v[t] = ld4(Vb + off);
    f.p[t] = ld4(Pb + off);
  }
}
template <int NT, int ACT>
__global__ __launch_bounds__(64 * kMlpWaves) __attribute__((amdgpu_waves_per_eu(2)))
void k_edge_mlp(EdgeHopArgs a) {
#pragma clang fp contract(off)
  constexpr int F = 16 * NT, T2 = 2 * NT;
  extern __shared__ __attribute__((aligned(16))) float smem[];
  const int w = wave_id();
  const int stride = gridDim.x * kMlpWaves;
  const int ch0 = blockIdx.x * kMlpWaves + w;
  if (a.step_inc && blockIdx.x == 0 && threadIdx.x == 0) *a.step_inc += 1;
  const bool full = MSW_EDGE_FULL && a.h1t == T2 && a.Pe;
  f32x4 H0[T2];
  int4 e0;
  auto chunk = [&](f32x4 (&H)[T2], const int4 e, const float* Wm, int ln, int g) __attribute__((always_inline)) {
    const bool ev = e.z >= 0;
    act_tiles<ACT, T2>(H, a.act1, a.slope1);
    f32x4 sv[NT];
    if (a.rest.n > 0) {
      run_mlp<T2, T2, NT, ACT>(H, sv, a.rest, Wm, ln, g);
    } else {
#pragma unroll
      for (int t = 0; t < NT; ++t) sv[t] = H[t];
    }
    mask_pad<ACT, NT>(sv, a.c.fl, g);
    if (a.normalize) normalize_s<NT>(sv);
    if (ev) store_row<NT>(a.s + (size_t)e.z * F, sv, NT, g);
  };
  auto run = [&](const float* Wm, auto fullc) __attribute__((always_inline)) {
    constexpr bool FULL = decltype(fullc)::value;
    if constexpr (FULL) {
      if (ch0 < a.nchunks) {
        const int ln = opaque_lane(), g = ln >> 4;
        chunk(H0, e0, Wm, ln, g);
      }
      for (int ch = ch0 + stride; ch < a.nchunks; ch += stride) {
        const int ln = opaque_lane(), g = ln >> 4, j = ln & 15;
        MlpFetch<NT> f;
        mlp_fetch_full<NT>(f, a, ch, true, j, g);
        f32x4 H[T2];
#pragma unroll
        for (int t = 0; t < T2; ++t) H[t] = (f.u[t] + f.v[t]) + f.p[t];
        chunk(H, f.e, Wm, ln, g);
      }
    } else {
      const int hs = 16 * a.h1t;
      const float* z = a.c.zrow;
      const int b1 = a.b1_off >= 0 ? a.b1_off : 0;
      for (int ch = ch0; ch < a.nchunks; ch += stride) {
        const int ln = opaque_lane(), g = ln >> 4, j = ln & 15;
        const int4 e = reinterpret_cast<const int4*>(a.chunks)[(size_t)ch * kRowsPerWave + j];
        const bool ev = e.z >= 0;
        const float* Ub = a.U + (size_t)(ev ? e.x : a.n0) * hs;
        const float* Vb = a.V + (size_t)(ev ? e.y : a.n0) * hs;
        const float* Pb = a.Pe && ev ? a.Pe + (size_t)e.z * hs : z;
        f32x4 H[T2];
#pragma unroll
        for (int t = 0; t < T2; ++t) {
          const int off = 16 * t + 4 * g;
          const bool on = t < a.h1t;
          const f32x4 u = ld4((on ? Ub : z) + off);
          const f32x4 v = ld4((on ? Vb : z) + off);
          const f32x4 pe = ld4((on ? Pb : z) + off);
          const f32x4 p = a.Pe ? pe : ld4(Wm + b1 + off);
          H[t] = on ? (u + v) + p : zero4();
        }
        chunk(H, e, Wm, ln, g);
      }
    }
  };
  if (a.reg.len > 0) stage_glds<kMlpWaves>(smem, a.c.W, a.reg, 0, a.reg.len);
  {
    const int lane = threadIdx.x & 63;
    MlpFetch<NT> f0;
    mlp_fetch_full<NT>(f0, a, ch0 < a.nchunks ? ch0 : 0, full && ch0 < a.nchunks, lane & 15, lane >> 4);
    e0 = f0.e;
#pragma unroll
    for (int t = 0; t < T2; ++t) H0[t] = (f0.u[t] + f0.v[t]) + f0.p[t];
  }
  if (a.reg.len > 0) __syncthreads();
  if (w >= 4)
    for (int k = 0; k < a.stagger; ++k) __builtin_amdgcn_s_sleep(32);
  if (a.reg.len > 0) {
    if (full)
      run(smem, std::true_type{});
    else
      run(smem, std::false_type{});
  } else if (full) {
    run(a.c.W, std::true_type{});
  } else {
    run(a.c.W, std::false_type{});
  }
}
```

### mswe-gnn_amd/csrc/kernels/k_encode.h

```cpp
#pragma once

template <int NT, int ACT, bool DEC, bool STREAM = false>
__global__ __launch_bounds__(kBlock) void k_encode(EncodeArgs a) {
  constexpr bool ST = STREAM && !DEC;
  constexpr int F = 16 * NT;
  extern __shared__ __attribute__((aligned(16))) float smem[];
  const int lane = threadIdx.x & 63, g = lane >> 4, j = lane & 15;
  MSW_MARK(a.c, 0);
  Common c = a.c;
  const int dstep = DEC ? a.dec.io->step : -1;
  if (!a.dec.on && a.io && blockIdx.x == 0 && threadIdx.x == 0) a.io->step += 1;
  const int nchunks = a.Npad / kRowsPerBlock;
  int staged = -1;
  for (int chunk = blockIdx.x; chunk < nchunks; chunk += gridDim.x) {
    const int rb = chunk * kRowsPerBlock;
    int s = 0;
    while (s + 1 < a.S && rb >= a.n0[s + 1]) ++s;
    const int n = rb + wave_id() * kRowsPerWave + j;
    const bool valid = (n - a.n0[s]) < a.ns[s];
    const int ext = a.c.perm ? a.c.perm[n] : n;
    const int xrow = a.x_internal ? (valid ? n : a.n0[s]) : (valid ? ext : 0);
    const float* xr = a.x + (size_t)xrow * a.c.nnf;
    const int nstat = a.c.nstat_raw;
    float raw[4], dyn[4];
    float wlv;
    EpiPre<NT> pre;
    f32x4 xu[NT];
    if (DEC) {
      load_row<NT>(xu, a.dec_in + (size_t)n * F, g);
      pre.ext = ext;
      pre.bc = a.dec.bc_slot[n];
#pragma unroll
      for (int k = 0; k < kMaxDyn; ++k) pre.xd[k] = k < c.dyn ? xr[nstat + k] : 0.f;
    }
#pragma unroll
    for (int r = 0; r < 4; ++r) {
      const int f = 4 * g + r;
      raw[r] = f < nstat ? xr[f] : 0.f;
      dyn[r] = f < a.c.dyn ? xr[nstat + f] : 0.f;
    }
    wlv = xr[nstat - 1] + xr[a.c.nnf - 2];
    if constexpr (kBcHoist<NT>) {
      if (DEC && dstep >= 0) {
        pre.step = dstep;
        bc_prefetch<NT, true>(pre, a.dec, c);
      }
    }
    MSW_MARK(c, 1);
    if constexpr (kStaged<NT>) {
      if (s != staged) {
        if (staged >= 0) __syncthreads();
        stage_glds(smem, a.c.W, a.sreg[s], 0, a.sreg[s].len);
        __syncthreads();
        staged = s;
      }
    }
    const float* Wl = kStaged<NT> ? (const float*)smem : c.W;
    if (DEC && dstep >= 0) {
      if constexpr (!kBcHoist<NT>) {
        pre.step = dstep;
        bc_prefetch<NT, true>(pre, a.dec, c);
      }
      float nd[kMaxDyn];
      decode_state<NT, ACT, true>(xu, a.dec, c, Wl, pre, n, valid, lane, g, nd);
#pragma unroll
      for (int r = 0; r < 4; ++r) dyn[r] = nd_column(nd, g, r, c.dyn);
      float hn = 0.f;
#pragma unroll
      for (int k = 0; k < kMaxDyn; ++k) hn = (k == c.dyn - 2) ? nd[k] : hn;
      wlv = xr[nstat - 1] + hn;
    }
    if (DEC && a.decode_only) continue;
    MSW_MARK(c, 2);
    f32x4 xs[NT];
    {
      f32x4 v;
#pragma unroll
      for (int r = 0; r < 4; ++r) v[r] = (c.with_wl && 4 * g + r == nstat) ? wlv : raw[r];
      const f32x4 in[1] = {v};
      run_mlp<1, NT, NT, ACT>(in, xs, a.stat, Wl, lane, g);
      mask_pad<ACT, NT>(xs, c.fl, g);
      if (valid) store_row<NT, ST>(a.xs + (size_t)n * F, xs, NT, g);
    }
    MSW_MARK(c, 5);
    if (s == 0) {
      f32x4 xd[NT];
      const f32x4 in[1] = {f32x4{dyn[0], dyn[1], dyn[2], dyn[3]}};
      run_mlp<1, NT, NT, ACT>(in, xd, a.dynm, Wl, lane, g);
      mask_pad<ACT, NT>(xd, c.fl, g);
      if (valid && a.xd) store_row<NT, ST>(a.xd + (size_t)n * F, xd, NT, g);
      MSW_MARK(c, 6);
      np_project<NT, ST>(xs, xd, a.np0, Wl, n, valid, lane, g);
    }
    MSW_MARK(c, 8);
    if (a.vu_a[s] >= 0) side_proj<NT, NT, ST>(xs, a.vu_h1t, Wl + a.vu_a[s], a.Vu, n, valid, lane, g);
  }
  MSW_MARK(c, 9);
}

template <int NT, int ACT>
__global__ __launch_bounds__(kBlock) void k_decode_fwd(DecodeArgs a) {
  constexpr int F = 16 * NT;
  const int lane = threadIdx.x & 63, g = lane >> 4, j = lane & 15;
  const int n = wave_row0() + j;
  if (wave_row0() >= a.Npad) return;
  const bool valid = n < a.Npad;
  const int nn = valid ? n : 0;
  EpiPre<NT> pre;
  f32x4 xu[NT];
  load_row<NT>(xu, a.in + (size_t)nn * F, g);
  const Common& c = a.c;
  pre.ext = valid ? c.perm[nn] : -1;
  pre.step = 0;
  pre.bc = -1;
  const float* xr = a.dec.X + (size_t)(pre.ext > 0 ? pre.ext : 0) * c.nnf + (c.nnf - c.dyn);
#pragma unroll
  for (int k = 0; k < kMaxDyn; ++k) pre.xd[k] = k < c.dyn ? xr[k] : 0.f;
  decode_rows<NT, ACT>(xu, a.dec, c, pre, nn, valid, lane, g);
}
```

### mswe-gnn_amd/csrc/kernels/k_hop.h

```cpp
#pragma once

template <int NT>
struct HopRows {
  Lanes L;
  f32x4 os[NT], sv[NT], inn[NT];
  EpiPre<NT> pre;
};
template <int NT, bool LAST>
__device__ __forceinline__ void hop_gather(HopRows<NT>& r, const HopArgs& a, const LaneRec& rec, int tile, int j,
                                           int g) {
  constexpr int F = 16 * NT;
  r.L = lanes_of(rec, tile, j, a.n0);
  load_row<NT>(r.os, a.in + r.L.sr * F, g);
  load_row<NT>(r.sv, a.s + r.L.p * F, g);
  load_row<NT>(r.inn, a.in + r.L.n * F, g);
  if constexpr (LAST) epi_prefetch<NT>(r.pre, a.epi, a.c, a.xs, r.L.n, g);
}
template <int NT, bool LAST>
__device__ __forceinline__ void hop_load(HopRows<NT>& r, const HopArgs& a, int tile, int j, int g) {
  hop_gather<NT, LAST>(r, a, load_rec(a.recs, tile, j), tile, j, g);
}
template <int NT, int ACT, bool LAST, bool LOOP>
__global__ __launch_bounds__((64 * hop_waves<NT, LOOP>())) void k_hop(HopArgs a) {
#pragma clang fp contract(off)
  constexpr int WV = hop_waves<NT, LOOP>();
  constexpr int F = 16 * NT;
  constexpr int XS = F + 4;
  __shared__ __attribute__((aligned(16))) float slab_all[WV][kRowsPerWave][XS];
  extern __shared__ __attribute__((aligned(16))) float smem[];
  const int lane = threadIdx.x & 63, g = lane >> 4, j = lane & 15, w = wave_id();
  const int stride = gridDim.x * WV;
  const int xb = logical_block(a.c);
  if (xb < 0) return;
  int tile = xb * WV + w;
  Common c = a.c;
  MSW_MARK(c, 0);
  f32x4 wf[NT][NT];
  load_filter<NT>(wf, c.W, a.filt_a, lane);
  float* slab = &slab_all[w][0][0];
  auto core = [&](const HopRows<NT>& r, int j, int lane, int g, f32x4 (&res)[NT]) {
    float* my = slab + j * XS;
    const Lanes& L = r.L;
    store_row<NT>(my, r.inn, NT, g);
    wave_lds_sync();
    f32x4 od[NT];
    load_row<NT>(od, slab + L.dl * XS, g);
    MSW_MARK(c, 4);
    put_message<NT>(my, r.os, od, r.sv, L.ev, a.grad, a.upwind, g);
    MSW_MARK(c, 6);
    f32x4 agg[NT];
    gather_messages<NT, XS>(agg, slab, L.q0, L.q1, g);
    MSW_MARK(c, 7);
#pragma unroll
    for (int t = 0; t < NT; ++t) res[t] = r.inn[t];
    apply_filter_regs<NT>(res, agg, a.filt_a, wf);
    MSW_MARK(c, 8);
  };
  auto finish = [&](f32x4 (&res)[NT], const HopRows<NT>& r, int lane, int g) {
    const Lanes& L = r.L;
    if constexpr (LAST) {
      node_epilogue<NT, ACT>(res, a.epi, c, r.pre, a.out, L.n, L.nv, lane, g);
    } else {
      if (L.nv) store_row<NT>(a.out + L.n * F, res, NT, g);
    }
  };
  if constexpr (!LOOP) {
    const bool live = tile < a.ntiles;
    HopRows<NT> r;
    hop_load<NT, LAST>(r, a, live ? tile : 0, j, g);
    MSW_MARK(c, 1);
    if constexpr (LAST && kStaged<NT>) stage_glds<WV>(smem, a.c.W, a.reg, 0, a.reg.len);
    f32x4 res[NT];
    if (live) core(r, j, lane, g, res);
    if constexpr (LAST && kStaged<NT>) {
      __syncthreads();
      c.W = smem;
    }
    MSW_MARK(c, 2);
    if (live) finish(res, r, lane, g);
  } else {
    if constexpr (LAST && kStaged<NT>) {
      stage_glds<WV>(smem, a.c.W, a.reg, 0, a.reg.len);
      __syncthreads();
      c.W = smem;
    }
    if (LAST) {
      for (; tile < a.ntiles; tile += stride) {
        const int ln = opaque_lane(), gg = ln >> 4, jj = ln & 15;
        HopRows<NT> q;
        hop_load<NT, LAST>(q, a, tile, jj, gg);
        f32x4 res[NT];
        core(q, jj, ln, gg, res);
        finish(res, q, ln, gg);
      }
    } else if (tile < a.ntiles) {
      HopRows<NT> q;
      hop_load<NT, LAST>(q, a, tile, j, g);
      int t1 = tile + stride;
      LaneRec rn = load_rec(a.recs, t1 < a.ntiles ? t1 : tile, j);
      for (;;) {
        const int ln = opaque_lane(), gg = ln >> 4, jj = ln & 15;
        const bool more = t1 < a.ntiles;
        HopRows<NT> qn;
        if (more) {
          hop_gather<NT, LAST>(qn, a, rn, t1, jj, gg);
          const int t2 = t1 + stride;
          rn = load_rec(a.recs, t2 < a.ntiles ? t2 : t1, jj);
        }
        f32x4 res[NT];
        core(q, jj, ln, gg, res);
        finish(res, q, ln, gg);
        if (!more) break;
        q = qn;
        t1 += stride;
      }
    }
  }
  MSW_MARK(c, 9);
}

constexpr int kRowHopWaves = 8;
constexpr int kRowDc = 3;
template <int NT>
__global__ __launch_bounds__(64 * kRowHopWaves) void k_hop_rows(HopArgs a) {
#pragma clang fp contract(off)
  constexpr int F = 16 * NT;
  constexpr int DC = NT >= 4 ? 2 : kRowDc;
  [[maybe_unused]] const int lane = threadIdx.x & 63;
  const int w = wave_id();
  const int stride = gridDim.x * kRowHopWaves;
  const int ntile = (a.nrows + kRowsPerWave - 1) / kRowsPerWave;
  f32x4 wf[NT][NT];
  load_filter<NT>(wf, a.c.W, a.filt_a, lane);
  for (int tile = blockIdx.x * kRowHopWaves + w; tile < ntile; tile += stride) {
    const int ln = opaque_lane(), g = ln >> 4, j = ln & 15;
    const int k = tile * kRowsPerWave + j;
    const bool valid = k < a.nrows;
    const int kc = valid ? k : 0;
    const int q0 = a.rptr[kc], q1 = valid ? a.rptr[kc + 1] : q0;
    const size_t n = (size_t)a.n0 + kc;
    f32x4 od[NT];
    load_row<NT>(od, a.in + n * F, g);
    const int deg = q1 - q0;
    int dmax = deg;
#pragma unroll
    for (int o = 1; o < 64; o <<= 1) dmax = max(dmax, __shfl_xor(dmax, o));
    float rd = 0.f;
#pragma unroll
    for (int t = 0; t < NT; ++t) rd += hsum(od[t]);
    const bool zd = row_sum(rd) != 0.f;
    f32x4 agg[NT];
#pragma unroll
    for (int t = 0; t < NT; ++t) agg[t] = zero4();
    for (int q = 0; q < dmax; q += DC) {
      int2 e[DC];
#pragma unroll
      for (int u = 0; u < DC; ++u)
        e[u] = q + u < deg ? a.redge[q0 + q + u] : int2{(int)n, 0};
      f32x4 os[DC][NT], sv[DC][NT];
#pragma unroll
      for (int u = 0; u < DC; ++u) {
        load_row<NT>(os[u], a.in + (size_t)e[u].x * F, g);
        load_row<NT>(sv[u], a.s + (size_t)e[u].y * F, g);
      }
#pragma unroll
      for (int u = 0; u < DC; ++u) {
        float rs = 0.f;
#pragma unroll
        for (int t = 0; t < NT; ++t) rs += hsum(os[u][t]);
        const bool act = (row_sum(rs) != 0.f) || zd;
        const bool has = q + u < deg;
#pragma unroll
        for (int t = 0; t < NT; ++t) {
          f32x4 gv;
          if (a.grad) {
            gv = od[t] - os[u][t];
            if (a.upwind) {
              gv.x = gv.x < 0.f ? 0.f : gv.x; gv.y = gv.y < 0.f ? 0.f : gv.y;
              gv.z = gv.z < 0.f ? 0.f : gv.z; gv.w = gv.w < 0.f ? 0.f : gv.w;
            }
          } else {
            gv = os[u][t];
          }
          const f32x4 m = act ? gv * sv[u][t] : zero4();
          const f32x4 sum = agg[t] + m;
          agg[t] = has ? sum : agg[t];
        }
      }
    }
    f32x4 res[NT];
#pragma unroll
    for (int t = 0; t < NT; ++t) res[t] = od[t];
    apply_filter_regs<NT>(res, agg, a.filt_a, wf);
    if (valid) store_row<NT, true>(a.out + n * F, res, NT, g);
  }
}

template <int NT>
__global__ __launch_bounds__(kBlock) void k_hop_split(HopArgs a) {
#pragma clang fp contract(off)
  constexpr int F = 16 * NT, TH = NT / 2, G = kWaves / 2;
  constexpr int XS = 16 * TH + 4;
  __shared__ __attribute__((aligned(16))) float slab_all[G][2][kRowsPerWave][XS];
  __shared__ __attribute__((aligned(16))) float hx[G][2][2 * TH][64];
  __shared__ __attribute__((aligned(16))) f32x4 ax[G][NT][64];
  const int lane = threadIdx.x & 63, g = lane >> 4, j = lane & 15, w = wave_id();
  const int grp = w / 2, r = w % 2, t0 = r * TH;
  const int xb = logical_block(a.c);
  if (xb < 0) return;
  const int tile = xb * G + grp;
  const bool live = tile < a.ntiles;
  MSW_MARK(a.c, 0);
  const Lanes L = lanes_of(load_rec(a.recs, live ? tile : 0, j), live ? tile : 0, j, a.n0);
  f32x4 os[TH], sv[TH], inn[TH];
#pragma unroll
  for (int t = 0; t < TH; ++t) {
    const int off = 16 * (t0 + t) + 4 * g;
    os[t] = ld4(a.in + L.sr * F + off);
    sv[t] = ld4(a.s + L.p * F + off);
    inn[t] = ld4(a.in + L.n * F + off);
  }
  f32x4 wf[TH][NT];
  {
    const int fa = a.filt_a >= 0 ? a.filt_a : 0;
#pragma unroll
    for (int to = 0; to < TH; ++to)
#pragma unroll
      for (int ti = 0; ti < NT; ++ti) wf[to][ti] = ld4(a.c.W + fa + ((size_t)((t0 + to) * NT + ti) * 64 + lane) * 4);
  }
  float* slab = &slab_all[grp][r][0][0];
  float* my = slab + j * XS;
#pragma unroll
  for (int t = 0; t < TH; ++t) st4(my + 16 * t + 4 * g, inn[t]);
  wave_lds_sync();
  f32x4 od[TH];
#pragma unroll
  for (int t = 0; t < TH; ++t) od[t] = ld4(slab + L.dl * XS + 16 * t + 4 * g);
#pragma unroll
  for (int t = 0; t < TH; ++t) {
    hx[grp][r][t][lane] = hsum(os[t]);
    hx[grp][r][TH + t][lane] = hsum(od[t]);
  }
  __syncthreads();
  float rs = 0.f, rd = 0.f;
#pragma unroll
  for (int q = 0; q < 2; ++q)
#pragma unroll
    for (int t = 0; t < TH; ++t) {
      rs += hx[grp][q][t][lane];
      rd += hx[grp][q][TH + t][lane];
    }
  const bool act = (row_sum(rs) != 0.f) || (row_sum(rd) != 0.f);
#pragma unroll
  for (int t = 0; t < TH; ++t) {
    f32x4 gv;
    if (a.grad) {
      gv = od[t] - os[t];
      if (a.upwind) {
        gv.x = gv.x < 0.f ? 0.f : gv.x; gv.y = gv.y < 0.f ? 0.f : gv.y;
        gv.z = gv.z < 0.f ? 0.f : gv.z; gv.w = gv.w < 0.f ? 0.f : gv.w;
      }
    } else {
      gv = os[t];
    }
    const f32x4 m = gv * sv[t];
    st4(my + 16 * t + 4 * g, (L.ev && act) ? m : zero4());
  }
  f32x4 agg[TH];
  gather_messages<TH, XS>(agg, slab, L.q0, L.q1, g);
#pragma unroll
  for (int t = 0; t < TH; ++t) ax[grp][t0 + t][lane] = agg[t];
  __syncthreads();
  f32x4 res[TH];
#pragma unroll
  for (int t = 0; t < TH; ++t) res[t] = inn[t];
  if (a.filt_a >= 0) {
    f32x4 full[NT], acc[TH];
#pragma unroll
    for (int ti = 0; ti < NT; ++ti) full[ti] = ax[grp][ti][lane];
#pragma unroll
    for (int to = 0; to < TH; ++to) acc[to] = zero4();
#pragma unroll
    for (int ti = 0; ti < NT; ++ti)
#pragma unroll
      for (int q = 0; q < 4; ++q)
#pragma unroll
        for (int to = 0; to < TH; ++to) acc[to] = MSW_MFMA(wf[to][ti][q], full[ti][q], acc[to]);
#pragma unroll
    for (int t = 0; t < TH; ++t) res[t] = res[t] + acc[t];
  } else {
#pragma unroll
    for (int t = 0; t < TH; ++t) res[t] = res[t] + agg[t];
  }
  if (live && L.nv) {
#pragma unroll
    for (int t = 0; t < TH; ++t) st4(a.out + L.n * F + 16 * (t0 + t) + 4 * g, res[t]);
  }
  MSW_MARK(a.c, 9);
}

template <int NT, int ACT, int P>
__device__ __forceinline__ void node_epilogue_coop(f32x4 (&res)[NT], const Epilogue& e, const Common& c,
                                                   const EpiPre<NT>& pre, float* out, int n, bool valid,
                                                   int r, int lane, int g, int j, float* b0, float* b1, int xw) {
#pragma clang fp contract(off)
  constexpr int F = 16 * NT, T2 = 2 * NT;
  if (e.post_act) {
    act_tiles<-1, NT>(res, e.post_act, e.post_slope);
    mask_pad<ACT, NT>(res, c.fl, g);
  }
  if (out && valid && r == 0) store_row<NT>(out + (size_t)n * F, res, NT, g);
  if (e.np.a_u >= 0 || e.np.a_v >= 0 || e.np.a_o >= 0) {
    if (e.np.h1t == T2)
      np_project_coop<NT, T2, P>(pre.xs, res, e.np, c.W, (size_t)n, valid, r, lane, g);
    else
      np_project_coop<NT, NT, P>(pre.xs, res, e.np, c.W, (size_t)n, valid, r, lane, g);
  }
  if (e.uu_a >= 0) {
    f32x4 in[T2];
#pragma unroll
    for (int t = 0; t < NT; ++t) {
      in[t] = pre.xs[t];
      in[NT + t] = res[t];
    }
    if (e.uu_h1t == T2)
      proj_store_part<T2, T2 / P>(in, c.W + e.uu_a, r, e.Uu, (size_t)n, T2, valid, lane, g);
    else
      proj_store_part<T2, NT / P>(in, c.W + e.uu_a, r, e.Uu, (size_t)n, NT, valid, lane, g);
  }
  if (e.dec.on) {
    const DecDesc& d = e.dec;
    f32x4 x0[NT], o[1];
#pragma unroll
    for (int t = 0; t < NT; ++t) x0[t] = res[t];
    act_tiles<-1, NT>(x0, d.pre_act, d.pre_slope);
    const MlpDev& m = d.dec;
    if (m.n == 1) {
      mfma_layer<NT, 1, ACT>(x0, o, m.l[0], c.W, lane, g);
    } else {
      f32x4 h[NT];
      {
        f32x4 p[NT / P];
        mfma_layer_sub<NT, NT / P, ACT>(x0, p, m.l[0], c.W, r * (NT / P), lane, g);
        coop_exchange<NT, P>(p, h, b1, xw, r, j, g);
      }
      for (int li = 1; li + 1 < m.n; ++li) {
        f32x4 p[NT / P];
        mfma_layer_sub<NT, NT / P, ACT>(h, p, m.l[li], c.W, r * (NT / P), lane, g);
        coop_exchange<NT, P>(p, h, (li & 1) ? b0 : b1, xw, r, j, g);
      }
      mfma_layer<NT, 1, ACT>(h, o, m.l[m.n - 1], c.W, lane, g);
    }
    if (r == 0) decode_tail<NT>(o, d, c, pre, n, valid, g);
  }
}

template <int NT, int ACT, int P>
__global__ __launch_bounds__(kBlock) void k_hop_coop(HopArgs a) {
#pragma clang fp contract(off)
  constexpr int F = 16 * NT, TS = NT / P;
  constexpr int XS = F + 4;
  constexpr int XW = 16 * NT + 4;
  constexpr int G = kWaves / P;
  __shared__ __attribute__((aligned(16))) float slab_all[kWaves][kRowsPerWave][XS];
  __shared__ __attribute__((aligned(16))) float xbuf[G][2][kRowsPerWave][XW];
  extern __shared__ __attribute__((aligned(16))) float smem[];
  const int lane = threadIdx.x & 63, g = lane >> 4, j = lane & 15, w = wave_id();
  const int grp = w / P, r = w % P;
  const int xb = logical_block(a.c);
  if (xb < 0) return;
  const int tile = xb * G + grp;
  const bool live = tile < a.ntiles;
  Common c = a.c;
  f32x4 wr[TS][NT];
  {
    const int fa = a.filt_a >= 0 ? a.filt_a : 0;
#pragma unroll
    for (int to = 0; to < TS; ++to)
#pragma unroll
      for (int ti = 0; ti < NT; ++ti) wr[to][ti] = ld4(c.W + fa + ((size_t)((r * TS + to) * NT + ti) * 64 + lane) * 4);
  }
  HopRows<NT> q;
  hop_load<NT, true>(q, a, live ? tile : 0, j, g);
  if constexpr (kStaged<NT>) stage_glds<kWaves>(smem, a.c.W, a.reg, 0, a.reg.len);
  const Lanes& L = q.L;
  float* slab = &slab_all[w][0][0];
  float* my = slab + j * XS;
  store_row<NT>(my, q.inn, NT, g);
  wave_lds_sync();
  f32x4 od[NT];
  load_row<NT>(od, slab + L.dl * XS, g);
  put_message<NT>(my, q.os, od, q.sv, L.ev, a.grad, a.upwind, g);
  f32x4 agg[NT];
  gather_messages<NT, XS>(agg, slab, L.q0, L.q1, g);
  f32x4 rs[TS];
#pragma unroll
  for (int t = 0; t < TS; ++t) rs[t] = ld4(a.in + L.n * F + 16 * (r * TS + t) + 4 * g);
  if (a.filt_a >= 0) {
    f32x4 acc[TS];
#pragma unroll
    for (int to = 0; to < TS; ++to) acc[to] = zero4();
#pragma unroll
    for (int ti = 0; ti < NT; ++ti)
#pragma unroll
      for (int rr = 0; rr < 4; ++rr)
#pragma unroll
        for (int to = 0; to < TS; ++to) acc[to] = MSW_MFMA(wr[to][ti][rr], agg[ti][rr], acc[to]);
#pragma unroll
    for (int t = 0; t < TS; ++t) rs[t] = rs[t] + acc[t];
  } else {
#pragma unroll
    for (int t = 0; t < TS; ++t) {
      f32x4 ag = zero4();
      for (int qq = L.q0; qq < L.q1; ++qq) ag = ag + ld4(slab + qq * XS + 16 * (r * TS + t) + 4 * g);
      rs[t] = rs[t] + ag;
    }
  }
  f32x4 res[NT];
  float* b0 = &xbuf[grp][0][0][0];
  float* b1 = &xbuf[grp][1][0][0];
  coop_exchange<NT, P>(rs, res, b0, XW, r, j, g);
  if constexpr (kStaged<NT>) c.W = smem;
  node_epilogue_coop<NT, ACT, P>(res, a.epi, c, q.pre, a.out, (int)L.n, live && L.nv, r, lane, g, j, b0, b1, XW);
}

template <int NT>
static const void* hop_coop_kernel(int prelu) {
  if constexpr (NT >= 2) return prelu ? (const void*)k_hop_coop<NT, 1, NT> : (const void*)k_hop_coop<NT, -1, NT>;
  return nullptr;
}
```

### mswe-gnn_amd/csrc/kernels/k_pool_epi.h

```cpp
#pragma once

template <int NT, bool LOOP>
__global__ __launch_bounds__((64 * waves_of<NT, LOOP>())) void k_pool(PoolArgs a) {
#pragma clang fp contract(off)
  constexpr int WV = waves_of<NT, LOOP>();
  constexpr int F = 16 * NT;
  extern __shared__ __attribute__((aligned(16))) float smem[];
  const int lane = threadIdx.x & 63, g = lane >> 4, j = lane & 15, w = wave_id();
  const int stride = gridDim.x * WV;
  const int xb = logical_block(a.c);
  if (xb < 0) return;
  int tile = xb * WV + w;
  Common c = a.c;
  MSW_MARK(c, 0);
  struct Rows {
    f32x4 acc[NT], xs[NT];
    size_t n;
    bool nv;
  };
  auto load = [&](Rows& r, int t, int j, int g) {
    const int i = 16 * t + j;
    r.nv = i < a.ns;
    r.n = (size_t)a.n0 + (r.nv ? i : 0);
    int4 rc = *reinterpret_cast<const int4*>(a.recs + 16 * t + j);
    const int2 ro = *reinterpret_cast<const int2*>(&a.recs[16 * t + j].cnt);
    asm volatile("" : "+v"(rc.x));
    const int cnt = ro.x, off = ro.y;
    const int c0 = cnt > 0 ? rc.x : (int)r.n;
    const int ci[kPoolInline] = {c0, cnt > 1 ? rc.y : c0, cnt > 2 ? rc.z : c0, cnt > 3 ? rc.w : c0};
    f32x4 x[kPoolInline][NT];
#pragma unroll
    for (int k = 0; k < kPoolInline; ++k) load_row<NT>(x[k], a.in + (size_t)ci[k] * F, g);
    load_row<NT>(r.xs, a.xs + r.n * F, g);
#pragma unroll
    for (int t2 = 0; t2 < NT; ++t2) r.acc[t2] = zero4();
#pragma unroll
    for (int k = 0; k < kPoolInline; ++k) {
#pragma unroll
      for (int t2 = 0; t2 < NT; ++t2) {
        const f32x4 s2 = r.acc[t2] + x[k][t2];
        r.acc[t2] = k < cnt ? s2 : r.acc[t2];
      }
    }
    for (int k = kPoolInline; k < cnt; ++k) {
      f32x4 y[NT];
      load_row<NT>(y, a.in + (size_t)a.child[off + k] * F, g);
#pragma unroll
      for (int t2 = 0; t2 < NT; ++t2) r.acc[t2] = r.acc[t2] + y[t2];
    }
    const float fc = (float)(cnt > 0 ? cnt : 1);
#pragma unroll
    for (int t2 = 0; t2 < NT; ++t2) r.acc[t2] = r.acc[t2] / fc;
  };
  if constexpr (!LOOP) {
    Rows r0;
    load(r0, tile < a.ntiles ? tile : 0, j, g);
    MSW_MARK(c, 1);
    if constexpr (kStaged<NT>) {
      stage_glds<WV>(smem, a.c.W, a.reg, 0, a.reg.len);
      __syncthreads();
      c.W = smem;
    }
    MSW_MARK(c, 2);
    if (tile < a.ntiles) np_project<NT>(r0.xs, r0.acc, a.np, c.W, r0.n, r0.nv, lane, g);
  } else {
    if constexpr (kStaged<NT>) {
      stage_glds<WV>(smem, a.c.W, a.reg, 0, a.reg.len);
      __syncthreads();
      c.W = smem;
    }
    for (; tile < a.ntiles; tile += stride) {
      const int ln = opaque_lane(), gg = ln >> 4, jj = ln & 15;
      Rows q;
      load(q, tile, jj, gg);
      np_project<NT>(q.xs, q.acc, a.np, c.W, q.n, q.nv, ln, gg);
    }
  }
  MSW_MARK(c, 9);
}

template <int NT, int P = 1, int WV = kWaves>
__global__ __launch_bounds__(64 * WV) void k_pool_edge(PoolArgs a) {
#pragma clang fp contract(off)
  constexpr int F = 16 * NT;
  constexpr int XS = F + 4;
  static_assert(WV % P == 0, "whole tiles per workgroup");
  __shared__ __attribute__((aligned(16))) float slab_all[WV][kRowsPerWave][XS];
  extern __shared__ __attribute__((aligned(16))) float smem[];
  const int lane = threadIdx.x & 63, g = lane >> 4, j = lane & 15, w = wave_id();
  const int xb = logical_block(a.c);
  if (xb < 0) return;
  int tile = xb * (WV / P) + w / P;
  const int rk = w % P;
  Common c = a.c;
  MSW_MARK(c, 0);
  struct Rows {
    Lanes L;
    f32x4 x[NT], xs[NT];
  };
  auto load = [&](Rows& r, int t, int j, int g) {
    r.L = lanes_of(load_rec(a.erecs, t, j), t, j, a.n0);
    load_row<NT>(r.x, a.in + r.L.sr * F, g);
    load_row<NT>(r.xs, a.xs + r.L.n * F, g);
  };
  float* slab = &slab_all[w][0][0];
  auto run = [&](const Rows& r, int j, int lane, int g) {
    const Lanes& L = r.L;
    store_row<NT>(slab + j * XS, r.x, NT, g);
    f32x4 acc[NT];
    gather_messages<NT, XS>(acc, slab, L.q0, L.q1, g);
    MSW_MARK(c, 7);
    const float cnt = (float)(L.q1 - L.q0 > 0 ? L.q1 - L.q0 : 1);
#pragma unroll
    for (int t = 0; t < NT; ++t) acc[t] = acc[t] / cnt;
    if constexpr (P == 1) {
      np_project<NT>(r.xs, acc, a.np, c.W, L.n, L.nv, lane, g);
    } else {
      if (a.np.h1t == 2 * NT) {
        np_project_coop<NT, 2 * NT, P>(r.xs, acc, a.np, c.W, L.n, L.nv, rk, lane, g);
      } else if constexpr (P <= NT) {
        np_project_coop<NT, NT, P>(r.xs, acc, a.np, c.W, L.n, L.nv, rk, lane, g);
      }
    }
  };
  Rows r0;
  load(r0, tile < a.ntiles ? tile : 0, j, g);
  MSW_MARK(c, 1);
  if constexpr (kStaged<NT>) {
    stage_glds<WV>(smem, a.c.W, a.reg, 0, a.reg.len);
    __syncthreads();
    c.W = smem;
  }
  MSW_MARK(c, 2);
  if (tile < a.ntiles) run(r0, j, lane, g);
  MSW_MARK(c, 9);
}

template <int NT, int ACT, bool LOOP>
__global__ __launch_bounds__((64 * waves_of<NT, LOOP>())) void k_epi(EpiArgs a) {
#pragma clang fp contract(off)
  constexpr int WV = waves_of<NT, LOOP>();
  constexpr int F = 16 * NT;
  extern __shared__ __attribute__((aligned(16))) float smem[];
  const int lane = threadIdx.x & 63, g = lane >> 4, j = lane & 15, w = wave_id();
  const int stride = gridDim.x * WV;
  const int xb = logical_block(a.c);
  if (xb < 0) return;
  int tile = xb * WV + w;
  Common c = a.c;
  MSW_MARK(c, 0);
  struct Rows {
    f32x4 res[NT];
    EpiPre<NT> pre;
    int n;
    bool nv;
  };
  auto load = [&](Rows& r, int t, int j, int g) {
    const int i = 16 * t + j;
    r.nv = i < a.ns;
    r.n = a.n0 + (r.nv ? i : 0);
    load_row<NT>(r.res, a.in + (size_t)r.n * F, g);
    epi_prefetch<NT>(r.pre, a.epi, a.c, a.xs, (size_t)r.n, g);
  };
  if constexpr (!LOOP) {
    Rows r0;
    load(r0, tile < a.ntiles ? tile : 0, j, g);
    MSW_MARK(c, 1);
    if constexpr (kStaged<NT>) {
      stage_glds<WV>(smem, a.c.W, a.reg, 0, a.reg.len);
      __syncthreads();
      c.W = smem;
    }
    MSW_MARK(c, 2);
    if (tile < a.ntiles) node_epilogue<NT, ACT>(r0.res, a.epi, c, r0.pre, a.out, r0.n, r0.nv, lane, g);
  } else {
    if constexpr (kStaged<NT>) {
      stage_glds<WV>(smem, a.c.W, a.reg, 0, a.reg.len);
      __syncthreads();
      c.W = smem;
    }
    if (tile < a.ntiles) {
      Rows q;
      load(q, tile, j, g);
      for (;;) {
        const int ln = opaque_lane(), gg = ln >> 4, jj = ln & 15;
        const int t1 = tile + stride;
        const bool more = t1 < a.ntiles;
        Rows qn;
        if (more) load(qn, t1, jj, gg);
        node_epilogue<NT, ACT>(q.res, a.epi, c, q.pre, a.out, q.n, q.nv, ln, gg);
        if (!more) break;
        q = qn;
        tile = t1;
      }
    }
  }
  MSW_MARK(c, 9);
}

template <int NT, int MODE>
__global__ __launch_bounds__(kBlock) void k_rowmlp(RowMlpArgs a) {
  const int lane = threadIdx.x & 63, g = lane >> 4;
  const int r0 = wave_row0();
  if (r0 >= a.R) return;
  const int row = r0 + (lane & 15);
  const bool valid = row < a.R;
  const float* xr = a.in + (size_t)(valid ? row : 0) * a.in_stride;
  constexpr int TI = MODE == 0 ? 1 : NT, TO = MODE == 0 ? NT : 2 * NT;
  f32x4 in[TI], out[TO];
#pragma unroll
  for (int t = 0; t < TI; ++t) {
    f32x4 v;
#pragma unroll
    for (int r = 0; r < 4; ++r) {
      const int f = 16 * t + 4 * g + r;
      v[r] = f < a.in_dim ? xr[f] : 0.f;
    }
    in[t] = v;
  }
  if (MODE == 0)
    run_mlp<TI, NT, TO, -1>(in, out, a.m, a.W, lane, g);
  else
    mfma_layer<TI, TO, -1>(in, out, a.m.l[0], a.W, lane, g);
  if (valid) store_row<TO>(a.out + (size_t)row * a.out_stride, out, a.out_tiles, g);
}
```

Before: 51.60 million.

## Hoist kernel-argument loads into SGPRs at kernel entry across GNN kernels

Adds an MSW_PIN macro that uses empty inline asm with "s" constraints to force many kernel arguments to be loaded into scalar registers at kernel entry. This is meant to issue the kernarg scalar loads early and overlap their latency with other work. It also replaces per-scale array lookups in the encoders with vectorised kernarg tables and copies RolloutIO by value, and moves the step_inc increment later. A waves_per_eu attribute is added to k_epi. The risks are higher SGPR pressure and scheduling changes, and the old path stays available behind a build variant.

```diff
diff --git a/mswe-gnn_amd/build_engine.py b/mswe-gnn_amd/build_engine.py
--- a/mswe-gnn_amd/build_engine.py
+++ b/mswe-gnn_amd/build_engine.py
@@ -47,7 +47,8 @@
     odir = os.path.join(HERE, "_obj" + (f"_{variant}" if variant else ""))
     extra = {"trace": ["-DMSW_TRACE"],
              "valubase": ["-DMSW_PRELU_MAX=0", "-DMSW_EDGE_FULL=0"],
-             "nostream": ["-DMSW_STREAM_ST=0"]}.get(variant, [])
+             "nostream": ["-DMSW_STREAM_ST=0"],
+             "lazyargs": ["-DMSW_ARGS_HOIST=0"]}.get(variant, [])
     os.makedirs(odir, exist_ok=True)
     os.makedirs(os.path.join(HERE, "lib"), exist_ok=True)
     out = lib_path(variant)
diff --git a/mswe-gnn_amd/csrc/kernels/k_base.h b/mswe-gnn_amd/csrc/kernels/k_base.h
--- a/mswe-gnn_amd/csrc/kernels/k_base.h
+++ b/mswe-gnn_amd/csrc/kernels/k_base.h
@@ -39,6 +39,70 @@
     q.w = (q.w == q.w) ? q.w : 0.f;
     sv[t] = q;
   }
+}
+
+#ifndef MSW_ARGS_HOIST
+#define MSW_ARGS_HOIST 1
+#endif
+#define MSW_PIN_OP_1(a) "s"(a)
+#define MSW_PIN_OP_2(a, ...) "s"(a), MSW_PIN_OP_1(__VA_ARGS__)
+#define MSW_PIN_OP_3(a, ...) "s"(a), MSW_PIN_OP_2(__VA_ARGS__)
+#define MSW_PIN_OP_4(a, ...) "s"(a), MSW_PIN_OP_3(__VA_ARGS__)
+#define MSW_PIN_OP_5(a, ...) "s"(a), MSW_PIN_OP_4(__VA_ARGS__)
+#define MSW_PIN_OP_6(a, ...) "s"(a), MSW_PIN_OP_5(__VA_ARGS__)
+#define MSW_PIN_OP_7(a, ...) "s"(a), MSW_PIN_OP_6(__VA_ARGS__)
+#define MSW_PIN_OP_8(a, ...) "s"(a), MSW_PIN_OP_7(__VA_ARGS__)
+#define MSW_PIN_OP_9(a, ...) "s"(a), MSW_PIN_OP_8(__VA_ARGS__)
+#define MSW_PIN_OP_10(a, ...) "s"(a), MSW_PIN_OP_9(__VA_ARGS__)
+#define MSW_PIN_OP_11(a, ...) "s"(a), MSW_PIN_OP_10(__VA_ARGS__)
+#define MSW_PIN_OP_12(a, ...) "s"(a), MSW_PIN_OP_11(__VA_ARGS__)
+#define MSW_PIN_OP_13(a, ...) "s"(a), MSW_PIN_OP_12(__VA_ARGS__)
+#define MSW_PIN_OP_14(a, ...) "s"(a), MSW_PIN_OP_13(__VA_ARGS__)
+#define MSW_PIN_OP_15(a, ...) "s"(a), MSW_PIN_OP_14(__VA_ARGS__)
+#define MSW_PIN_OP_16(a, ...) "s"(a), MSW_PIN_OP_15(__VA_ARGS__)
+#define MSW_PIN_OP_17(a, ...) "s"(a), MSW_PIN_OP_16(__VA_ARGS__)
+#define MSW_PIN_OP_18(a, ...) "s"(a), MSW_PIN_OP_17(__VA_ARGS__)
+#define MSW_PIN_OP_19(a, ...) "s"(a), MSW_PIN_OP_18(__VA_ARGS__)
+#define MSW_PIN_OP_20(a, ...) "s"(a), MSW_PIN_OP_19(__VA_ARGS__)
+#define MSW_PIN_OP_21(a, ...) "s"(a), MSW_PIN_OP_20(__VA_ARGS__)
+#define MSW_PIN_OP_22(a, ...) "s"(a), MSW_PIN_OP_21(__VA_ARGS__)
+#define MSW_PIN_OP_23(a, ...) "s"(a), MSW_PIN_OP_22(__VA_ARGS__)
+#define MSW_PIN_OP_24(a, ...) "s"(a), MSW_PIN_OP_23(__VA_ARGS__)
+#define MSW_PIN_OP_25(a, ...) "s"(a), MSW_PIN_OP_24(__VA_ARGS__)
+#define MSW_PIN_OP_26(a, ...) "s"(a), MSW_PIN_OP_25(__VA_ARGS__)
+#define MSW_PIN_OP_27(a, ...) "s"(a), MSW_PIN_OP_26(__VA_ARGS__)
+#define MSW_PIN_OP_28(a, ...) "s"(a), MSW_PIN_OP_27(__VA_ARGS__)
+#define MSW_PIN_OP_29(a, ...) "s"(a), MSW_PIN_OP_28(__VA_ARGS__)
+#define MSW_PIN_OP_30(a, ...) "s"(a), MSW_PIN_OP_29(__VA_ARGS__)
+#define MSW_PIN_SEL( \
+    _1, _2, _3, _4, _5, _6, _7, _8, _9, _10, _11, _12, _13, _14, _15, _16, _17, _18, _19, _20, _21, \
+    _22, _23, _24, _25, _26, _27, _28, _29, _30, NAME, ...) \
+  NAME
+#define MSW_PIN_OPS(...) \
+  MSW_PIN_SEL( \
+      __VA_ARGS__, MSW_PIN_OP_30, MSW_PIN_OP_29, MSW_PIN_OP_28, MSW_PIN_OP_27, MSW_PIN_OP_26, \
+      MSW_PIN_OP_25, MSW_PIN_OP_24, MSW_PIN_OP_23, MSW_PIN_OP_22, MSW_PIN_OP_21, MSW_PIN_OP_20, \
+      MSW_PIN_OP_19, MSW_PIN_OP_18, MSW_PIN_OP_17, MSW_PIN_OP_16, MSW_PIN_OP_15, MSW_PIN_OP_14, \
+      MSW_PIN_OP_13, MSW_PIN_OP_12, MSW_PIN_OP_11, MSW_PIN_OP_10, MSW_PIN_OP_9, MSW_PIN_OP_8, \
+      MSW_PIN_OP_7, MSW_PIN_OP_6, MSW_PIN_OP_5, MSW_PIN_OP_4, MSW_PIN_OP_3, MSW_PIN_OP_2, \
+      MSW_PIN_OP_1) \
+  (__VA_ARGS__)
+#define MSW_PIN(...)                                                      \
+  do {                                                                    \
+    if constexpr (MSW_ARGS_HOIST) asm volatile("" ::MSW_PIN_OPS(__VA_ARGS__)); \
+  } while (0)
+#define MSW_PIN_IF(cond, x, other) ((cond) ? (int)(x) : (int)(other))
+#define MSW_ARGS_EPI_SW(e) (e).np.a_u, (e).np.a_v, (e).np.a_o, (e).np.h1t, (e).uu_a, (e).dec.on
+#define MSW_ARGS_EPI_REST(e) (e).post_act, (e).post_slope, (e).uu_h1t
+#define MSW_ARGS_MLP(m)                                                                                        \
+  (m).n, (m).l[0].a_off, (m).l[0].b_off, (m).l[0].slope, (m).l[1].a_off, (m).l[1].b_off, (m).l[1].slope,       \
+      (m).l[2].a_off, (m).l[2].b_off, (m).l[2].slope, (m).l[3].a_off, (m).l[3].b_off, (m).l[3].slope
+template <int N>
+using i32xN = int __attribute__((ext_vector_type(N)));
+template <int N>
+__device__ __forceinline__ i32xN<N> kernarg_vec(const void* p) {
+  typedef i32xN<N> __attribute__((aligned(4))) V;
+  return *reinterpret_cast<const V*>(p);
 }
 
 __device__ __forceinline__ int wave_id() { return threadIdx.x >> 6; }
@@ -240,8 +304,8 @@
   float bck[kMaxDyn];
 };
 template <int NT, bool BYCOL = false>
-__device__ __forceinline__ void bc_prefetch(EpiPre<NT>& p, const DecDesc& d, const Common& c) {
-  const RolloutIO* io = d.io;
+__device__ __forceinline__ void bc_prefetch(EpiPre<NT>& p, const RolloutIO& iov, const Common& c) {
+  const RolloutIO* io = &iov;
   const bool on = p.bc >= 0 && p.step + 1 < io->bc_tstride;
   const float* bp = on ? io->bc + (size_t)p.bc * c.p * io->bc_tstride + p.step + 1 : c.zrow;
   const int ts = on ? io->bc_tstride : 0;
diff --git a/mswe-gnn_amd/csrc/kernels/k_coop_edge.h b/mswe-gnn_amd/csrc/kernels/k_coop_edge.h
--- a/mswe-gnn_amd/csrc/kernels/k_coop_edge.h
+++ b/mswe-gnn_amd/csrc/kernels/k_coop_edge.h
@@ -351,6 +351,22 @@
   extern __shared__ __attribute__((aligned(16))) float smem[];
   const int lane = threadIdx.x & 63, g = lane >> 4, j = lane & 15, w = wave_id();
   const int grp = w / P, r = w % P;
+  if constexpr (FUSE == 1) {
+    if constexpr (LST != 0)
+      MSW_PIN(MSW_ARGS_EDGE(a), a.pool.slots, a.pool.in, MSW_ARGS_EPI_SW(a.epi));
+    else
+      MSW_PIN(MSW_ARGS_EDGE(a), a.pool.slots, a.pool.in);
+  } else if constexpr (FUSE == 2) {
+    if constexpr (LST != 0)
+      MSW_PIN(MSW_ARGS_EDGE(a), a.pool.parent, a.pool.cpad, a.pool.Uu, a.pool.Vu, a.pool.xc, a.pool.skip, a.pool.h1t,
+              MSW_ARGS_EPI_SW(a.epi));
+    else
+      MSW_PIN(MSW_ARGS_EDGE(a), a.pool.parent, a.pool.cpad, a.pool.Uu, a.pool.Vu, a.pool.xc, a.pool.skip, a.pool.h1t);
+  } else if constexpr (LST != 0) {
+    MSW_PIN(MSW_ARGS_EDGE(a), MSW_ARGS_EDGE_ROWS(a), MSW_ARGS_EPI_SW(a.epi));
+  } else {
+    MSW_PIN(MSW_ARGS_EDGE(a), MSW_ARGS_EDGE_ROWS(a));
+  }
   const int xb = logical_block(a.c);
   if (xb < 0) return;
   const int tile = xb * G + grp;
@@ -370,6 +386,11 @@
       edge_unpool_load<NT, LST>(q, uin, a, live ? tile : 0, j, g, r);
     else
       edge_hop_load<NT, LST, FULL>(q, a, live ? tile : 0, j, g);
+    if constexpr (FUSE != 0)
+      MSW_PIN(MSW_ARGS_EDGE_STAGE(a), MSW_ARGS_EDGE_CHAIN(a), a.pool.np.a_u, a.pool.np.a_v, a.pool.np.a_o, a.pool.np.h1t);
+    else
+      MSW_PIN(MSW_ARGS_EDGE_STAGE(a), MSW_ARGS_EDGE_CHAIN(a));
+    if constexpr (LST != 0) MSW_PIN(MSW_ARGS_EPI_REST(a.epi));
     const bool split = a.reg.split < a.reg_nf;
     stage_glds<kWaves>(smem, a.c.W, a.reg, 0, a.reg.split);
     __syncthreads();
@@ -530,6 +551,16 @@
   extern __shared__ __attribute__((aligned(16))) float smem[];
   const int lane = threadIdx.x & 63, g = lane >> 4, j = lane & 15, w = wave_id();
   const int grp = w / P, r = w % P;
+  if constexpr (FUSE == 1) {
+    if constexpr (LST != 0)
+      MSW_PIN(MSW_ARGS_EDGE(a), a.pool.slots, a.pool.in, MSW_ARGS_EPI_SW(a.epi));
+    else
+      MSW_PIN(MSW_ARGS_EDGE(a), a.pool.slots, a.pool.in);
+  } else if constexpr (LST != 0) {
+    MSW_PIN(MSW_ARGS_EDGE(a), MSW_ARGS_EDGE_ROWS(a), MSW_ARGS_EPI_SW(a.epi));
+  } else {
+    MSW_PIN(MSW_ARGS_EDGE(a), MSW_ARGS_EDGE_ROWS(a));
+  }
   const int xb = logical_block(a.c);
   if (xb < 0) return;
   const int tile0 = xb * G + grp;
@@ -558,6 +589,12 @@
   else
     edge_hop_load<NT, LST>(q, a, tile, j, g);
   const Lanes& L = q.L;
+  if constexpr (FUSE != 0)
+    MSW_PIN(a.wdirect, MSW_ARGS_EDGE_STAGE(a), MSW_ARGS_EDGE_CHAIN(a), a.pool.np.a_u, a.pool.np.a_v, a.pool.np.a_o,
+            a.pool.np.h1t);
+  else
+    MSW_PIN(a.wdirect, MSW_ARGS_EDGE_STAGE(a), MSW_ARGS_EDGE_CHAIN(a));
+  if constexpr (LST != 0) MSW_PIN(MSW_ARGS_EPI_REST(a.epi));
   if (a.reg.len > 0 && !a.wdirect) stage_glds<kWaves>(smem, c.W, a.reg, 0, a.reg.len);
   auto rest = [&](const float* Wm, auto fullc) __attribute__((always_inline)) {
     constexpr bool FULL = decltype(fullc)::value;
diff --git a/mswe-gnn_amd/csrc/kernels/k_coop_encode.h b/mswe-gnn_amd/csrc/kernels/k_coop_encode.h
--- a/mswe-gnn_amd/csrc/kernels/k_coop_encode.h
+++ b/mswe-gnn_amd/csrc/kernels/k_coop_encode.h
@@ -92,17 +92,30 @@
   extern __shared__ __attribute__((aligned(16))) float smem[];
   const int lane = threadIdx.x & 63, g = lane >> 4, j = lane & 15, w = wave_id();
   const int grp = w / P, r = w % P;
+  constexpr bool TAB = !DEC;
+  constexpr bool SCAL = MSW_ARGS_HOIST && !DEC && NT == 4;
+  EncTables<kStaged<NT>> tb{};
+  if constexpr (MSW_ARGS_HOIST && TAB && !SCAL) tb = enc_tables<kStaged<NT>>(a);
+  if constexpr (DEC)
+    MSW_PIN(MSW_ARGS_ENC(a), MSW_ARGS_ENC_DEC(a));
+  else if constexpr (kStaged<NT>)
+    MSW_PIN(MSW_ARGS_ENC(a), MSW_ARGS_ENC_TAB(tb), MSW_ARGS_ENC_REG(tb));
+  else
+    MSW_PIN(MSW_ARGS_ENC(a), MSW_ARGS_ENC_N(a));
   MSW_MARK(a.c, 0);
   Common c = a.c;
-  const int dstep = DEC ? a.dec.io->step : -1;
+  RolloutIO iocopy{};
+  if constexpr (DEC && MSW_ARGS_HOIST) iocopy = *a.dec.io;
+  const RolloutIO& iov = (DEC && !MSW_ARGS_HOIST) ? *a.dec.io : iocopy;
+  const int dstep = DEC ? iov.step : -1;
   if (!a.dec.on && a.io && blockIdx.x == 0 && threadIdx.x == 0) a.io->step += 1;
   const int rb = blockIdx.x * (G * kRowsPerWave);
-  int s = 0;
-  while (s + 1 < a.S && rb >= a.n0[s + 1]) ++s;
+  const EncScale sc = SCAL ? enc_scale_scalars(a, rb) : TAB ? enc_scale(a, tb, rb) : enc_scale(a, rb);
+  const int s = sc.s;
   const int n = rb + grp * kRowsPerWave + j;
-  const bool valid = (n - a.n0[s]) < a.ns[s];
+  const bool valid = (n - sc.n0) < sc.ns;
   const int ext = a.c.perm ? a.c.perm[n] : n;
-  const int xrow = a.x_internal ? (valid ? n : a.n0[s]) : (valid ? ext : 0);
+  const int xrow = a.x_internal ? (valid ? n : sc.n0) : (valid ? ext : 0);
   const float* xr = a.x + (size_t)xrow * a.c.nnf;
   const int nstat = a.c.nstat_raw;
   float raw[4], dyn[4];
@@ -126,14 +139,15 @@
   }
   wlv = xr[nstat - 1] + xr[a.c.nnf - 2];
   if constexpr (kBcHoist<NT>) {
+    if constexpr (DEC) MSW_PIN(iov.step, iov.bc, iov.bc_tstride, iov.type_bc);
     if (DEC && dstep >= 0) {
       pre.step = dstep;
-      bc_prefetch<NT>(pre, a.dec, c);
+      bc_prefetch<NT>(pre, iov, c);
     }
   }
   MSW_MARK(c, 1);
   if constexpr (kStaged<NT>) {
-    stage_glds<WV>(smem, a.c.W, a.sreg[s], 0, a.sreg[s].len);
+    stage_glds<WV>(smem, a.c.W, sc.reg, 0, sc.reg.len);
     __syncthreads();
   }
   const float* Wl = kStaged<NT> ? (const float*)smem : c.W;
@@ -153,7 +167,7 @@
     dec_mlp.load(a.dec.dec, Wl, r, lane, g);
     if constexpr (!kBcHoist<NT>) {
       pre.step = dstep;
-      bc_prefetch<NT>(pre, a.dec, c);
+      bc_prefetch<NT>(pre, iov, c);
     }
     float nd[kMaxDyn];
     {
@@ -196,11 +210,11 @@
       np_project_coop<NT, NT, P, kEncProjAhead>(xs, xd, a.np0, Wl, n, valid, r, lane, g);
   }
   MSW_MARK(c, 8);
-  if (a.vu_a[s] >= 0) {
+  if (sc.vu_a >= 0) {
     if (a.vu_h1t == T2)
-      proj_store_part<NT, T2 / P, kEncProjAhead>(xs, Wl + a.vu_a[s], r, a.Vu, n, T2, valid, lane, g);
+      proj_store_part<NT, T2 / P, kEncProjAhead>(xs, Wl + sc.vu_a, r, a.Vu, n, T2, valid, lane, g);
     else
-      proj_store_part<NT, NT / P, kEncProjAhead>(xs, Wl + a.vu_a[s], r, a.Vu, n, NT, valid, lane, g);
+      proj_store_part<NT, NT / P, kEncProjAhead>(xs, Wl + sc.vu_a, r, a.Vu, n, NT, valid, lane, g);
   }
   MSW_MARK(c, 9);
 }
diff --git a/mswe-gnn_amd/csrc/kernels/k_edge.h b/mswe-gnn_amd/csrc/kernels/k_edge.h
--- a/mswe-gnn_amd/csrc/kernels/k_edge.h
+++ b/mswe-gnn_amd/csrc/kernels/k_edge.h
@@ -236,6 +236,14 @@
     store_row<NT>(a.out + L.n * F, res, NT, g);
   }
 }
+#define MSW_ARGS_EDGE(a)                                                                                    \
+  (a).c.xcd, (a).ntiles, (a).recs, (a).n0, (a).step_inc, (a).c.W, (a).c.zrow, (a).filt_a, (a).Pe, (a).h1t, \
+      (a).xs, (a).own_zero, (a).skip, (a).grad, (a).upwind, (a).last
+#define MSW_ARGS_EDGE_ROWS(a) (a).U, (a).V, (a).in
+#define MSW_ARGS_EDGE_STAGE(a) (a).reg.off, (a).reg.len, (a).reg.split, (a).reg_nf
+#define MSW_ARGS_EDGE_ACT(a, act) MSW_PIN_IF((act) < 0, (a).c.fl, (a).ntiles)
+#define MSW_ARGS_EDGE_DEC(a) (a).c.nnf, (a).c.dyn, (a).c.p, (a).c.nstat_raw
+#define MSW_ARGS_EDGE_CHAIN(a) (a).b1_off, (a).act1, (a).slope1, (a).normalize, MSW_ARGS_MLP((a).rest)
 template <int NT, int ACT, bool LOOP, int LST>
 __global__ __launch_bounds__((64 * edge_waves<NT, LOOP, LST>())) __attribute__((amdgpu_waves_per_eu(edge_eu<NT, LOOP, LST>())))
 void k_edge_hop(EdgeHopArgs a) {
@@ -245,6 +253,23 @@
   extern __shared__ __attribute__((aligned(16))) float smem[];
   const int lane = threadIdx.x & 63, g = lane >> 4, j = lane & 15, w = wave_id();
   const int stride = gridDim.x * WV;
+  if constexpr (LOOP && NT == 4) {
+    if constexpr (LST != 0)
+      MSW_PIN(stride, a.c.xcd, a.ntiles, a.recs, a.n0, a.step_inc, a.c.W, a.filt_a, a.reg.off, a.reg.len, a.reg.split,
+              MSW_ARGS_EDGE_DEC(a));
+    else
+      MSW_PIN(stride, a.c.xcd, a.ntiles, a.recs, a.n0, a.step_inc, a.c.W, a.filt_a, a.reg.off, a.reg.len, a.reg.split);
+  } else if constexpr (LOOP) {
+    if constexpr (LST != 0)
+      MSW_PIN(stride, a.c.xcd, a.ntiles, a.recs, a.n0, a.step_inc, a.c.W, a.filt_a, a.Pe, a.h1t, a.own_zero, a.skip, a.grad,
+              a.upwind, a.last, a.reg.off, a.reg.len, a.reg.split, MSW_ARGS_EPI_SW(a.epi), MSW_ARGS_EDGE_DEC(a));
+    else
+      MSW_PIN(MSW_ARGS_EDGE(a), MSW_ARGS_EDGE_ROWS(a), MSW_ARGS_EDGE_STAGE(a));
+  } else if constexpr (LST != 0) {
+    MSW_PIN(MSW_ARGS_EDGE(a), MSW_ARGS_EDGE_ROWS(a), MSW_ARGS_EPI_SW(a.epi), MSW_ARGS_EDGE_ACT(a, ACT), MSW_ARGS_EDGE_DEC(a));
+  } else {
+    MSW_PIN(MSW_ARGS_EDGE(a), MSW_ARGS_EDGE_ROWS(a), MSW_ARGS_EDGE_ACT(a, ACT));
+  }
   const int xb = logical_block(a.c);
   if (xb < 0) return;
   int tile = xb * WV + w;
@@ -260,6 +285,10 @@
       const bool live = tile < a.ntiles;
       EdgeHopRows<NT> r;
       edge_hop_load<NT, LST, FULL>(r, a, live ? tile : 0, j, g);
+      if constexpr (LST != 0)
+        MSW_PIN(MSW_ARGS_EDGE_STAGE(a), MSW_ARGS_EDGE_CHAIN(a), MSW_ARGS_EPI_REST(a.epi));
+      else
+        MSW_PIN(MSW_ARGS_EDGE_STAGE(a), MSW_ARGS_EDGE_CHAIN(a));
       MSW_MARK(c, 1);
       const bool split = kStaged<NT> && a.reg.split < a.reg_nf;
       const float* Wm = c.W;
@@ -358,7 +387,14 @@
   const int w = wave_id();
   const int stride = gridDim.x * kMlpWaves;
   const int ch0 = blockIdx.x * kMlpWaves + w;
-  if (a.step_inc && blockIdx.x == 0 && threadIdx.x == 0) *a.step_inc += 1;
+  if constexpr (NT == 4)
+    MSW_PIN(stride, a.nchunks, a.chunks, a.c.W, a.U, a.V, a.Pe, a.h1t, a.reg.off, a.reg.len);
+  else
+    MSW_PIN(stride, a.nchunks, a.chunks, a.n0, a.step_inc, a.c.W, a.c.zrow, a.U, a.V, a.Pe, a.h1t, a.reg.off, a.reg.len,
+            a.stagger, a.s);
+  if constexpr (!MSW_ARGS_HOIST) {
+    if (a.step_inc && blockIdx.x == 0 && threadIdx.x == 0) *a.step_inc += 1;
+  }
   const bool full = MSW_EDGE_FULL && a.h1t == T2 && a.Pe;
   f32x4 H0[T2];
   int4 e0;
@@ -427,6 +463,9 @@
 #pragma unroll
     for (int t = 0; t < T2; ++t) H0[t] = (f0.u[t] + f0.v[t]) + f0.p[t];
   }
+  if constexpr (MSW_ARGS_HOIST) {
+    if (a.step_inc && blockIdx.x == 0 && threadIdx.x == 0) *a.step_inc += 1;
+  }
   if (a.reg.len > 0) __syncthreads();
   if (w >= 4)
     for (int k = 0; k < a.stagger; ++k) __builtin_amdgcn_s_sleep(32);
diff --git a/mswe-gnn_amd/csrc/kernels/k_encode.h b/mswe-gnn_amd/csrc/kernels/k_encode.h
--- a/mswe-gnn_amd/csrc/kernels/k_encode.h
+++ b/mswe-gnn_amd/csrc/kernels/k_encode.h
@@ -1,25 +1,102 @@
 #pragma once
 
+struct EncScale {
+  int s, n0, ns, vu_a;
+  WReg reg;
+};
+template <bool STAGED>
+struct EncTables {
+  i32xN<8> n0, ns, vu;
+  i32xN<16> ra;
+  i32xN<8> rb;
+};
+template <>
+struct EncTables<false> {
+  i32xN<8> n0, ns, vu;
+};
+static_assert(kMaxScales == 8 && sizeof(WReg) == 12, "EncTables: eight scales, {off, len, split} regions");
+template <bool STAGED>
+__device__ __forceinline__ EncTables<STAGED> enc_tables(const EncodeArgs& a) {
+  if constexpr (STAGED)
+    return EncTables<true>{kernarg_vec<8>(a.n0), kernarg_vec<8>(a.ns), kernarg_vec<8>(a.vu_a), kernarg_vec<16>(a.sreg),
+                           kernarg_vec<8>(reinterpret_cast<const int*>(a.sreg) + 16)};
+  else
+    return EncTables<false>{kernarg_vec<8>(a.n0), kernarg_vec<8>(a.ns), kernarg_vec<8>(a.vu_a)};
+}
+__device__ __forceinline__ EncScale enc_scale(const EncodeArgs& a, int rb) {
+  int s = 0;
+  while (s + 1 < a.S && rb >= a.n0[s + 1]) ++s;
+  return EncScale{s, a.n0[s], a.ns[s], a.vu_a[s], a.sreg[s]};
+}
+template <bool STAGED>
+__device__ __forceinline__ EncScale enc_scale(const EncodeArgs& a, const EncTables<STAGED>& t, int rb) {
+  if constexpr (!MSW_ARGS_HOIST) return enc_scale(a, rb);
+  EncScale e{0, t.n0[0], t.ns[0], t.vu[0], WReg{0, 0, 0}};
+  if constexpr (STAGED) e.reg = WReg{t.ra[0], t.ra[1], 0};
+#pragma unroll
+  for (int k = 1; k < kMaxScales; ++k) {
+    const bool in = k < a.S && rb >= t.n0[k];
+    e.s = in ? k : e.s;
+    e.n0 = in ? t.n0[k] : e.n0;
+    e.ns = in ? t.ns[k] : e.ns;
+    e.vu_a = in ? t.vu[k] : e.vu_a;
+    if constexpr (STAGED) {
+      const int off = 3 * k < 16 ? t.ra[3 * k < 16 ? 3 * k : 0] : t.rb[3 * k >= 16 ? 3 * k - 16 : 0];
+      const int len = 3 * k + 1 < 16 ? t.ra[3 * k + 1 < 16 ? 3 * k + 1 : 0] : t.rb[3 * k + 1 >= 16 ? 3 * k + 1 - 16 : 0];
+      e.reg.off = in ? off : e.reg.off;
+      e.reg.len = in ? len : e.reg.len;
+    }
+  }
+  return e;
+}
+#define MSW_ARGS_ENC(a)                                                                                       \
+  (a).Npad, (a).S, (a).x, (a).x_internal, (a).c.perm, (a).c.nnf, (a).c.nstat_raw, (a).c.dyn, (a).c.W, (a).io, \
+      (a).dec.on
+#define MSW_ARGS_ENC_DEC(a) (a).dec.io, (a).dec_in, (a).dec.bc_slot
+#define MSW_ARGS_ENC_TAB(t) (t).n0, (t).ns, (t).vu
+#define MSW_ARGS_ENC_REG(t) (t).ra, (t).rb
+#define MSW_ARGS_ENC_N(a)                                                                                  \
+  (a).n0[0], (a).n0[1], (a).n0[2], (a).n0[3], (a).n0[4], (a).n0[5], (a).n0[6], (a).n0[7], (a).ns[0], (a).ns[1], \
+      (a).ns[2], (a).ns[3], (a).ns[4], (a).ns[5], (a).ns[6], (a).ns[7]
+__device__ __forceinline__ EncScale enc_scale_scalars(const EncodeArgs& a, int rb) {
+  EncScale e{0, a.n0[0], a.ns[0], 0, WReg{0, 0, 0}};
+#pragma unroll
+  for (int k = 1; k < kMaxScales; ++k) {
+    const bool in = k < a.S && rb >= a.n0[k];
+    e.s = in ? k : e.s;
+    e.n0 = in ? a.n0[k] : e.n0;
+    e.ns = in ? a.ns[k] : e.ns;
+  }
+  e.vu_a = a.vu_a[e.s];
+  return e;
+}
 template <int NT, int ACT, bool DEC, bool STREAM = false>
 __global__ __launch_bounds__(kBlock) void k_encode(EncodeArgs a) {
   constexpr bool ST = STREAM && !DEC;
   constexpr int F = 16 * NT;
   extern __shared__ __attribute__((aligned(16))) float smem[];
   const int lane = threadIdx.x & 63, g = lane >> 4, j = lane & 15;
+  if constexpr (DEC)
+    MSW_PIN(MSW_ARGS_ENC(a), MSW_ARGS_ENC_DEC(a));
+  else
+    MSW_PIN(MSW_ARGS_ENC(a));
   MSW_MARK(a.c, 0);
   Common c = a.c;
-  const int dstep = DEC ? a.dec.io->step : -1;
+  RolloutIO iocopy{};
+  if constexpr (DEC && MSW_ARGS_HOIST) iocopy = *a.dec.io;
+  const RolloutIO& iov = (DEC && !MSW_ARGS_HOIST) ? *a.dec.io : iocopy;
+  const int dstep = DEC ? iov.step : -1;
   if (!a.dec.on && a.io && blockIdx.x == 0 && threadIdx.x == 0) a.io->step += 1;
   const int nchunks = a.Npad / kRowsPerBlock;
   int staged = -1;
   for (int chunk = blockIdx.x; chunk < nchunks; chunk += gridDim.x) {
     const int rb = chunk * kRowsPerBlock;
-    int s = 0;
-    while (s + 1 < a.S && rb >= a.n0[s + 1]) ++s;
+    const EncScale sc = enc_scale(a, rb);
+    const int s = sc.s;
     const int n = rb + wave_id() * kRowsPerWave + j;
-    const bool valid = (n - a.n0[s]) < a.ns[s];
+    const bool valid = (n - sc.n0) < sc.ns;
     const int ext = a.c.perm ? a.c.perm[n] : n;
-    const int xrow = a.x_internal ? (valid ? n : a.n0[s]) : (valid ? ext : 0);
+    const int xrow = a.x_internal ? (valid ? n : sc.n0) : (valid ? ext : 0);
     const float* xr = a.x + (size_t)xrow * a.c.nnf;
     const int nstat = a.c.nstat_raw;
     float raw[4], dyn[4];
@@ -41,16 +118,17 @@
     }
     wlv = xr[nstat - 1] + xr[a.c.nnf - 2];
     if constexpr (kBcHoist<NT>) {
+      if constexpr (DEC) MSW_PIN(iov.step, iov.bc, iov.bc_tstride, iov.type_bc);
       if (DEC && dstep >= 0) {
         pre.step = dstep;
-        bc_prefetch<NT, true>(pre, a.dec, c);
+        bc_prefetch<NT, true>(pre, iov, c);
       }
     }
     MSW_MARK(c, 1);
     if constexpr (kStaged<NT>) {
       if (s != staged) {
         if (staged >= 0) __syncthreads();
-        stage_glds(smem, a.c.W, a.sreg[s], 0, a.sreg[s].len);
+        stage_glds(smem, a.c.W, sc.reg, 0, sc.reg.len);
         __syncthreads();
         staged = s;
       }
@@ -59,7 +137,7 @@
     if (DEC && dstep >= 0) {
       if constexpr (!kBcHoist<NT>) {
         pre.step = dstep;
-        bc_prefetch<NT, true>(pre, a.dec, c);
+        bc_prefetch<NT, true>(pre, iov, c);
       }
       float nd[kMaxDyn];
       decode_state<NT, ACT, true>(xu, a.dec, c, Wl, pre, n, valid, lane, g, nd);
@@ -93,7 +171,7 @@
       np_project<NT, ST>(xs, xd, a.np0, Wl, n, valid, lane, g);
     }
     MSW_MARK(c, 8);
-    if (a.vu_a[s] >= 0) side_proj<NT, NT, ST>(xs, a.vu_h1t, Wl + a.vu_a[s], a.Vu, n, valid, lane, g);
+    if (sc.vu_a >= 0) side_proj<NT, NT, ST>(xs, a.vu_h1t, Wl + sc.vu_a, a.Vu, n, valid, lane, g);
   }
   MSW_MARK(c, 9);
 }
@@ -102,6 +180,8 @@
 __global__ __launch_bounds__(kBlock) void k_decode_fwd(DecodeArgs a) {
   constexpr int F = 16 * NT;
   const int lane = threadIdx.x & 63, g = lane >> 4, j = lane & 15;
+  MSW_PIN(a.Npad, a.in, a.c.perm, a.dec.X, a.c.nnf, a.c.dyn, a.c.W, a.dec.pre_act, a.dec.pre_slope, a.dec.resw_off,
+          a.dec.y, a.dec.dec.l[0].tin, MSW_ARGS_MLP(a.dec.dec));
   const int n = wave_row0() + j;
   if (wave_row0() >= a.Npad) return;
   const bool valid = n < a.Npad;
diff --git a/mswe-gnn_amd/csrc/kernels/k_hop.h b/mswe-gnn_amd/csrc/kernels/k_hop.h
--- a/mswe-gnn_amd/csrc/kernels/k_hop.h
+++ b/mswe-gnn_amd/csrc/kernels/k_hop.h
@@ -20,6 +20,10 @@
 __device__ __forceinline__ void hop_load(HopRows<NT>& r, const HopArgs& a, int tile, int j, int g) {
   hop_gather<NT, LAST>(r, a, load_rec(a.recs, tile, j), tile, j, g);
 }
+#define MSW_ARGS_HOP(a) \
+  (a).c.xcd, (a).ntiles, (a).recs, (a).n0, (a).in, (a).s, (a).out, (a).c.W, (a).filt_a, (a).grad, (a).upwind
+#define MSW_ARGS_HOP_LAST(a) \
+  (a).xs, (a).reg.off, (a).reg.len, (a).reg.split, (a).last, (a).c.perm, (a).c.nnf, (a).c.dyn, MSW_ARGS_EPI_SW((a).epi)
 template <int NT, int ACT, bool LAST, bool LOOP>
 __global__ __launch_bounds__((64 * hop_waves<NT, LOOP>())) void k_hop(HopArgs a) {
 #pragma clang fp contract(off)
@@ -30,6 +34,13 @@
   extern __shared__ __attribute__((aligned(16))) float smem[];
   const int lane = threadIdx.x & 63, g = lane >> 4, j = lane & 15, w = wave_id();
   const int stride = gridDim.x * WV;
+  if constexpr (LAST && LOOP) {
+    MSW_PIN(stride, a.c.xcd, a.ntiles, a.recs, a.n0, a.c.W, a.filt_a, a.reg.off, a.reg.len, a.reg.split);
+  } else if constexpr (LAST) {
+    MSW_PIN(MSW_ARGS_HOP(a), MSW_ARGS_HOP_LAST(a));
+  } else {
+    MSW_PIN(MSW_ARGS_HOP(a));
+  }
   const int xb = logical_block(a.c);
   if (xb < 0) return;
   int tile = xb * WV + w;
@@ -37,6 +48,7 @@
   MSW_MARK(c, 0);
   f32x4 wf[NT][NT];
   load_filter<NT>(wf, c.W, a.filt_a, lane);
+  if constexpr (MSW_ARGS_HOIST && LAST && LOOP) __builtin_amdgcn_sched_barrier(0);
   float* slab = &slab_all[w][0][0];
   auto core = [&](const HopRows<NT>& r, int j, int lane, int g, f32x4 (&res)[NT]) {
     float* my = slab + j * XS;
@@ -68,6 +80,7 @@
     const bool live = tile < a.ntiles;
     HopRows<NT> r;
     hop_load<NT, LAST>(r, a, live ? tile : 0, j, g);
+    if constexpr (LAST) MSW_PIN(MSW_ARGS_EPI_REST(a.epi));
     MSW_MARK(c, 1);
     if constexpr (LAST && kStaged<NT>) stage_glds<WV>(smem, a.c.W, a.reg, 0, a.reg.len);
     f32x4 res[NT];
@@ -129,6 +142,7 @@
   [[maybe_unused]] const int lane = threadIdx.x & 63;
   const int w = wave_id();
   const int stride = gridDim.x * kRowHopWaves;
+  MSW_PIN(stride, a.nrows, a.rptr, a.redge, a.n0, a.in, a.s, a.out, a.c.W, a.filt_a, a.grad, a.upwind);
   const int ntile = (a.nrows + kRowsPerWave - 1) / kRowsPerWave;
   f32x4 wf[NT][NT];
   load_filter<NT>(wf, a.c.W, a.filt_a, lane);
@@ -206,6 +220,7 @@
   __shared__ __attribute__((aligned(16))) f32x4 ax[G][NT][64];
   const int lane = threadIdx.x & 63, g = lane >> 4, j = lane & 15, w = wave_id();
   const int grp = w / 2, r = w % 2, t0 = r * TH;
+  MSW_PIN(MSW_ARGS_HOP(a));
   const int xb = logical_block(a.c);
   if (xb < 0) return;
   const int tile = xb * G + grp;
@@ -367,6 +382,7 @@
   extern __shared__ __attribute__((aligned(16))) float smem[];
   const int lane = threadIdx.x & 63, g = lane >> 4, j = lane & 15, w = wave_id();
   const int grp = w / P, r = w % P;
+  MSW_PIN(MSW_ARGS_HOP(a), MSW_ARGS_HOP_LAST(a));
   const int xb = logical_block(a.c);
   if (xb < 0) return;
   const int tile = xb * G + grp;
@@ -382,6 +398,7 @@
   }
   HopRows<NT> q;
   hop_load<NT, true>(q, a, live ? tile : 0, j, g);
+  MSW_PIN(MSW_ARGS_EPI_REST(a.epi));
   if constexpr (kStaged<NT>) stage_glds<kWaves>(smem, a.c.W, a.reg, 0, a.reg.len);
   const Lanes& L = q.L;
   float* slab = &slab_all[w][0][0];
diff --git a/mswe-gnn_amd/csrc/kernels/k_pool_epi.h b/mswe-gnn_amd/csrc/kernels/k_pool_epi.h
--- a/mswe-gnn_amd/csrc/kernels/k_pool_epi.h
+++ b/mswe-gnn_amd/csrc/kernels/k_pool_epi.h
@@ -8,6 +8,9 @@
   extern __shared__ __attribute__((aligned(16))) float smem[];
   const int lane = threadIdx.x & 63, g = lane >> 4, j = lane & 15, w = wave_id();
   const int stride = gridDim.x * WV;
+  MSW_PIN(MSW_PIN_IF(LOOP, stride, a.ntiles), a.np.U, a.np.V, a.np.O,
+          a.c.xcd, a.ntiles, a.recs, a.n0, a.ns, a.in, a.xs, a.child, a.c.W, a.reg.off, a.reg.len, a.reg.split,
+          a.np.a_u, a.np.a_v, a.np.a_o, a.np.h1t);
   const int xb = logical_block(a.c);
   if (xb < 0) return;
   int tile = xb * WV + w;
@@ -88,6 +91,8 @@
   __shared__ __attribute__((aligned(16))) float slab_all[WV][kRowsPerWave][XS];
   extern __shared__ __attribute__((aligned(16))) float smem[];
   const int lane = threadIdx.x & 63, g = lane >> 4, j = lane & 15, w = wave_id();
+  MSW_PIN(a.c.xcd, a.ntiles, a.erecs, a.n0, a.in, a.xs, a.c.W, a.reg.off, a.reg.len, a.reg.split, a.np.a_u, a.np.a_v,
+          a.np.a_o, a.np.h1t);
   const int xb = logical_block(a.c);
   if (xb < 0) return;
   int tile = xb * (WV / P) + w / P;
@@ -136,14 +141,24 @@
   MSW_MARK(c, 9);
 }
 
+template <int NT, bool LOOP>
+constexpr int epi_eu() { return NT == 2 && !LOOP ? 5 : 1; }
 template <int NT, int ACT, bool LOOP>
-__global__ __launch_bounds__((64 * waves_of<NT, LOOP>())) void k_epi(EpiArgs a) {
+__global__ __launch_bounds__((64 * waves_of<NT, LOOP>())) __attribute__((amdgpu_waves_per_eu(epi_eu<NT, LOOP>())))
+void k_epi(EpiArgs a) {
 #pragma clang fp contract(off)
   constexpr int WV = waves_of<NT, LOOP>();
   constexpr int F = 16 * NT;
   extern __shared__ __attribute__((aligned(16))) float smem[];
   const int lane = threadIdx.x & 63, g = lane >> 4, j = lane & 15, w = wave_id();
   const int stride = gridDim.x * WV;
+  if constexpr (ACT < 0)
+    MSW_PIN(MSW_PIN_IF(LOOP, stride, a.ntiles), a.c.xcd, a.ntiles, a.n0, a.ns, a.in, a.xs, a.c.W, a.reg.off, a.reg.len,
+            a.reg.split);
+  else
+    MSW_PIN(MSW_PIN_IF(LOOP, stride, a.ntiles), MSW_PIN_IF(LOOP, a.max_blocks, a.ntiles),
+            MSW_PIN_IF(LOOP, a.fit_blocks, a.ntiles), a.c.xcd, a.ntiles, a.n0, a.ns, a.in, a.xs, a.out, a.c.W, a.reg.off,
+            a.reg.len, a.reg.split, a.c.perm, a.c.nnf, a.c.dyn, MSW_ARGS_EPI_SW(a.epi));
   const int xb = logical_block(a.c);
   if (xb < 0) return;
   int tile = xb * WV + w;
```

New measurement: 54.05 million, median of 6. 1.05x the previous value.
